# whaiproject/BetaZero

Hardware: AMD Instinct MI355X
Metric: selfplay_games_per_s (higher is better)
Workload: dtype bf16

## Files before the change

betazero_amd/_lib.py:

```python
import ctypes as C
import os

HERE = os.path.dirname(os.path.abspath(__file__))
SO = os.environ.get("BZ_HIP_SO") or os.path.join(HERE, "libbz_hip.so")
ABI_VERSION = 7

BZ_OK, BZ_EINVAL, BZ_EILLEGAL_MOVE, BZ_EHIP, BZ_ENOMEM, BZ_ENOGPU, BZ_ESTATE = range(7)
GAME_TTT, GAME_REVERSI, GAME_REVERSI6, GAME_REVERSI4 = 0, 1, 2, 3
EVAL_UNIFORM, EVAL_HASH, EVAL_NET_F32, EVAL_NET_BF16, EVAL_EXTERNAL, EVAL_NET_FP8, EVAL_MLP_F32, EVAL_MLP_BF16 = range(8)
ST_RUNNING, ST_TERMINAL, ST_ILLEGAL, ST_MUST_PASS = range(4)
PASS_ACTION = 64
ENGINE_REUSE_SUBTREE = 1
ENGINE_EVAL_CACHE = 2
ENGINE_EVAL_CACHE_CARRY = 4
ENGINE_LEAVES_SHIFT = 8
ENGINE_LEAVES_MASK = 31 << ENGINE_LEAVES_SHIFT
PROBE_OPS = ("expf_spec", "logf_spec", "tanhf_spec", "fsqrt", "fdiv", "u01_spec", "hash_logit", "hash_value", "gamma_spec")
PROBE_HOST, PROBE_DEVICE = 0, 1
PROBE_MAP, PROBE_SWEEP = 0, 1
PROF_SLOTS = ("tower", "stem", "heads", "select", "expand_backup", "search_fused", "play", "env_step")
COUNTER_NAMES = ("n_sims", "n_path_nodes", "n_child_scored", "n_edges_backed", "n_expanded",
                 "n_child_written", "n_env_steps", "n_net_leaves", "n_cache_hits", "n_cache_hits_prev", "n_collisions")

u64, u32, i32, i64, vp = C.c_uint64, C.c_uint32, C.c_int32, C.c_int64, C.c_void_p
# ... 87 lines not shown
    "bz_reversi_legal_batch": (i32, [vp, vp, i64, vp, vp]),
    "bz_reversi_score_batch": (i32, [vp, vp, i64, vp, vp, vp]),
    "bz_ttt_step_batch": (i32, [vp, vp, vp, vp, i64, vp, vp, vp, vp, vp, vp]),
    "bz_reversi_minimax": (i32, [u64, u64, i32, i32, C.POINTER(i32), C.POINTER(i32)]),
    "bz_ttt_minimax": (i32, [u32, u32, i32, C.POINTER(i32), C.POINTER(i32)]),
    "bz_reversi_minimax_batch": (i32, [vp, vp, vp, i64, i32, i32, vp, vp, vp]),
    "bz_ttt_minimax_batch": (i32, [vp, vp, vp, vp, i64, vp, vp, vp]),
    "bz_augment_d4_batch": (i32, [vp, vp, vp, i64, i32, i32, vp, vp, vp, vp, vp]),
    "bz_net_update": (i32, [vp, vp, vp]),
    "bz_net_param_count": (i64, [i32, i32, i32]),
    "bz_net_workspace_bytes": (i64, [i32, i32, i32, i32]),
    "bz_net_create": (i32, [i32, i32, i32, i32, vp, vp, i64, vp, C.POINTER(vp)]),
    "bz_net_destroy": (i32, [vp]),
    "bz_net_forward_f32": (i32, [vp, vp, vp, i32, vp, vp, vp]),
    "bz_net_forward_bf16": (i32, [vp, vp, vp, i32, vp, vp, vp]),
    "bz_net_forward_fp8": (i32, [vp, vp, vp, i32, vp, vp, vp]),
    "bz_sym_index": (u32, [u64, u64, u64]),
    "bz_sym_board": (i32, [u64, i32, i32, C.POINTER(u64)]),
    "bz_sym_action_map": (i32, [i32, i32, vp]),
    "bz_net_sym_scratch_bytes": (i64, [i64]),
    "bz_net_forward_sym": (i32, [vp, i32, vp, vp, i32, i32, i32, u64, vp, i64, vp, vp, vp]),
    "bz_net_forward_sym_counted": (i32, [vp, i32, vp, vp, i32, vp, i32, i32, u64, vp, vp, vp]),
    "bz_net_forward_counted": (i32, [vp, i32, vp, vp, i32, vp, vp, vp, vp]),
    "bz_net_set_adaptive_shape": (i32, [vp, i32]),
    "bz_net_shape_tally": (i32, [vp, vp, vp]),
    "bz_net_set_tile_map": (i32, [vp, i32]),
    "bz_mlp_param_count": (i64, [i32]),
    "bz_mlp_workspace_bytes": (i64, [i32, i32]),
    "bz_mlp_create": (i32, [i32, i32, vp, vp, i64, vp, C.POINTER(vp)]),
    "bz_mlp_destroy": (i32, [vp]),
    "bz_mlp_update": (i32, [vp, vp, vp]),
    "bz_mlp_forward_f32": (i32, [vp, vp, vp, i32, vp, vp]),
    "bz_mlp_forward_bf16": (i32, [vp, vp, vp, i32, vp, vp]),
    "bz_mlp_forward_states_f32": (i32, [vp, vp, i32, vp, vp]),
    "bz_mlp_forward_states_bf16": (i32, [vp, vp, i32, vp, vp]),
    "bz_mlp_train_workspace_bytes": (i64, [i32, i32]),
    "bz_mlp_train_step": (i32, [vp, vp, vp, vp, vp, vp, vp, vp, i32, C.POINTER(MlpAdam), vp, i64, vp, vp, vp, vp]),
    "bz_engine_workspace_bytes": (i64, [C.POINTER(EngineCfg)]),
    "bz_engine_create": (i32, [C.POINTER(EngineCfg), vp, i64, C.POINTER(vp)]),
    "bz_engine_destroy": (i32, [vp]),
    "bz_engine_get_layout": (i32, [vp, C.POINTER(EngineLayout)]),
    "bz_engine_set_net": (i32, [vp, vp]),
    "bz_engine_set_mlp": (i32, [vp, vp]),
    "bz_engine_debug_set_search_seq": (i32, [vp, C.c_uint32]),
    "bz_engine_set_eval_symmetry": (i32, [vp, i32, u64]),
    "bz_engine_reset_games": (i32, [vp, vp]),
    "bz_engine_set_roots": (i32, [vp, vp, vp, vp, vp]),
    "bz_engine_search": (i32, [vp, vp]),
    "bz_engine_root_begin": (i32, [vp, vp]),
    "bz_engine_select": (i32, [vp, u32, vp]),
    "bz_engine_evaluate": (i32, [vp, vp]),
    "bz_engine_expand_backup": (i32, [vp, vp]),
    "bz_engine_root_noise": (i32, [vp, vp]),
    "bz_engine_root_stats": (i32, [vp, vp]),
    "bz_engine_play": (i32, [vp, i32, vp]),
    "bz_engine_gumbel_bytes": (i64, [C.POINTER(EngineCfg), i32]),
    "bz_engine_set_gumbel": (i32, [vp, i32, C.c_float, C.c_float, C.c_float, vp, i64, vp]),
    "bz_gumbel_considered_visits": (i32, [i32, i32, vp]),
    "bz_engine_playout_cap_bytes": (i64, [C.POINTER(EngineCfg)]),
    "bz_engine_set_playout_cap": (i32, [vp, i32, u32, vp, i64, vp]),
    "bz_playout_cap_budget": (i32, [u64, u64, u32, i32, i32, u32]),
    "bz_engine_set_forced_playouts": (i32, [vp, C.c_float, i32, vp]),
    "bz_engine_forced_playouts_check": (i32, [C.POINTER(EngineCfg), C.c_float]),
    "bz_forced_prune": (i32, [vp, vp, vp, i32, C.c_float, C.c_float, vp]),
    "bz_engine_gumbel_interior_bytes": (i64, [C.POINTER(EngineCfg)]),
    "bz_engine_set_gumbel_interior": (i32, [vp, i32, vp, i64, vp]),
    "bz_gumbel_interior_pick": (i32, [vp, vp, vp, i32, C.c_float, C.c_float, C.c_float, vp, vp]),
    "bz_engine_fpu_bytes": (i64, [C.POINTER(EngineCfg)]),
    "bz_engine_fpu_check": (i32, [C.POINTER(EngineCfg), C.c_float, C.c_float]),
    "bz_engine_set_fpu": (i32, [vp, i32, C.c_float, C.c_float, vp, i64, vp]),
    "bz_fpu_mass": (u32, [vp, vp, i32]),
    "bz_fpu_value": (C.c_float, [vp, vp, i32, C.c_float, C.c_float]),
    "bz_engine_solver_bytes": (i64, [C.POINTER(EngineCfg)]),
    "bz_engine_solver_check": (i32, [C.POINTER(EngineCfg)]),
    "bz_engine_set_solver": (i32, [vp, i32, vp, i64, vp]),
    "bz_engine_root_proven": (i32, [vp, vp, vp, vp, vp]),
    "bz_solver_node": (i32, [vp, i32]),
    "bz_solver_pick": (i32, [vp, vp, i32, i32, C.c_uint64]),
    "bz_engine_early_stop_bytes": (i64, [C.POINTER(EngineCfg)]),
    "bz_engine_early_stop_check": (i32, [C.POINTER(EngineCfg)]),
    "bz_engine_set_early_stop": (i32, [vp, i32, i32, vp, i64, vp]),
    "bz_engine_stopped": (i32, [vp, vp, vp]),
    "bz_early_stop_decided": (i32, [vp, i32, u32]),
    "bz_engine_surprise_bytes": (i64, [C.POINTER(EngineCfg)]),
    "bz_engine_set_surprise": (i32, [vp, vp, i64, vp]),
    "bz_engine_pack_surprise": (i32, [vp, vp, i64, i32, vp]),
    "bz_surprise_kl": (i32, [vp, vp, i32, vp]),
    "bz_surprise_resample_workspace_bytes": (i64, [i64]),
    "bz_surprise_resample": (i32, [vp, vp, vp, vp, vp, i64, C.c_float, u64, vp, i64, vp, vp, i64, vp, vp]),
    "bz_surprise_count": (i32, [C.c_float, C.c_float, C.c_float, u64, i64, i32, u64, u64, C.POINTER(i32)]),
    "bz_engine_search_value_bytes": (i64, [C.POINTER(EngineCfg)]),
    "bz_engine_set_search_value": (i32, [vp, vp, i64, vp]),
    "bz_engine_pack_search_value": (i32, [vp, vp, i64, i32, vp]),
    "bz_root_value": (i32, [vp, vp, i32, vp]),
    "bz_value_targets": (i32, [vp, vp, vp, vp, vp, i64, C.c_float, C.c_float, vp, vp, vp]),
    "bz_value_targets_segment": (i32, [vp, vp, vp, i32, C.c_float, C.c_float, vp]),
    "bz_merge_group": (i32, [vp, vp, vp, vp, vp, i32, i32, vp, vp, vp, vp, vp, vp]),
    "bz_merge_workspace_bytes": (i64, [i64, i32]),
    "bz_merge_positions": (i32, [C.POINTER(MergeRows), i64, i32, vp, vp, vp, vp, vp, vp, vp, i64, C.POINTER(MergeRows), vp, vp]),
    "bz_engine_ownership_bytes": (i64, [C.POINTER(EngineCfg)]),
    "bz_engine_set_ownership": (i32, [vp, vp, i64, vp]),
    "bz_engine_pack_ownership": (i32, [vp, vp, vp, i64, i32, vp]),
    "bz_ownership_row": (i32, [u64, u64, i32, vp, vp]),
    "bz_engine_resign_bytes": (i64, [C.POINTER(EngineCfg)]),
    "bz_engine_set_resign": (i32, [vp, C.c_float, i32, u32, vp, i64, vp]),
    "bz_engine_resign_rows": (i32, [vp, vp, vp, vp, vp, vp]),
    "bz_resign_step": (i32, [C.c_float, C.c_float, i32, i32, vp]),
    "bz_resign_playout": (i32, [u64, u64, u32]),
    "bz_engine_root_store_bytes": (i64, [C.POINTER(EngineCfg), i32, i32]),
    "bz_engine_set_root_store": (i32, [vp, vp, i64, i32, i32, vp]),
    "bz_engine_root_policy": (i32, [vp, vp, vp, vp]),
    "bz_engine_status": (i32, [vp, vp, C.POINTER(i32), C.POINTER(i64), C.POINTER(i32)]),
    "bz_mcts_select": (i32, [vp, u32, vp]),
    "bz_mcts_expand_backup": (i32, [vp, vp]),
    "bz_selfplay_run": (i32, [vp, i32, vp]),
    "bz_engines_step": (i32, [C.POINTER(vp), C.POINTER(vp), i32, i32, i32]),
    "bz_engines_search": (i32, [C.POINTER(vp), C.POINTER(vp), i32, i32]),
    "bz_match_workspace_bytes": (i64, [i32, i32, i32]),
    "bz_match_create": (i32, [i32, i32, i32, vp, i64, C.POINTER(vp)]),
    "bz_match_destroy": (i32, [vp]),
    "bz_match_get_layout": (i32, [vp, C.POINTER(MatchLayout)]),
    "bz_match_begin": (i32, [vp, u64, i32, vp]),
    "bz_match_ply": (i32, [vp, vp, vp, vp, vp, vp]),
    "bz_match_header": (i32, [vp, vp, C.POINTER(MatchHdr)]),
    "bz_match_opening_index": (i32, [u64, u64, i32, i32, C.POINTER(i32)]),
    "bz_engine_reset_counters": (i32, [vp, vp]),
    "bz_engine_sum_counters": (i32, [vp, vp]),
    "bz_examples_packed_bytes": (i64, [i32, i64]),
    "bz_engine_pack_examples": (i32, [vp, vp, i64, i64, i32, vp]),
    "bz_stream_overlap_probe": (i32, [vp, vp, i32, i32, C.POINTER(C.c_float)]),
    "bz_spec_probe": (i32, [i32, i32, i32, vp, vp, i64, u64, u64, vp, vp]),
    "bz_train_wf_bytes": (i64, [i32, i32]),
    "bz_train_positions_per_workgroup": (i32, [i32]),
    "bz_train_mask_bytes": (i64, [i32, i32, i32]),
    "bz_train_pack_weights": (i32, [vp, i32, i32, vp, vp, vp]),
    "bz_train_tower_fwd": (i32, [vp, vp, vp, i32, i32, i32, vp, vp, vp]),
    "bz_train_tower_bwd": (i32, [vp, vp, vp, vp, i32, i32, i32, vp, vp]),
    "bz_train_wgrad_splits": (i32, [i32, i32, i32]),
    "bz_train_wgrad_bias_rows": (i32, [i32, i32]),
    "bz_train_wgrad": (i32, [vp, vp, i32, i32, i32, i32, vp, vp, vp]),
    "bz_train_ends_sizes": (i32, [i32, i32, C.POINTER(i32)]),
    "bz_train_stem_fwd": (i32, [vp, i32, vp, vp, i32, vp, vp]),
    "bz_train_stem_wgrad": (i32, [vp, vp, vp, i32, i32, vp, vp]),
    "bz_train_heads": (i32, [vp, vp, i32, i32, i32, C.POINTER(TrainHeadParams), vp, vp, vp, vp, vp, vp]),
    "bz_train_heads_vt": (i32, [vp, vp, vp, i32, i32, i32, C.POINTER(TrainHeadParams), vp, vp, vp, vp, vp, vp]),
    "bz_train_heads_own": (i32, [vp, vp, C.POINTER(TrainOwn), i32, i32, i32, C.POINTER(TrainHeadParams), vp, vp, vp, vp, vp, vp]),
    "bz_train_heads_own_vt": (i32, [vp, vp, vp, C.POINTER(TrainOwn), i32, i32, i32, C.POINTER(TrainHeadParams), vp, vp, vp, vp, vp, vp]),
    "bz_train_own_finish": (i32, [C.POINTER(TrainOwn), i32, i32, vp, vp, vp, vp, C.POINTER(TrainOwnAdam), vp]),
    "bz_train_heads_wgrad": (i32, [vp, vp, vp, i32, i32, vp, vp]),
    "bz_train_finish": (i32, [C.POINTER(TrainPartials), C.POINTER(TrainTensors), i32, i32, i32, i32, vp, C.POINTER(TrainAdam), vp]),
    "bz_train_optim_partials": (i32, []),
    "bz_train_optim_hyper": (i32, [C.c_float, C.c_float, C.c_float, C.c_float, C.c_float, C.c_float, C.POINTER(C.c_float)]),
    "bz_train_optim_step": (i32, [C.POINTER(TrainTensors), C.POINTER(TrainOptim), i32, i32, i32, vp]),
    "bz_profile_enable": (i32, [i32]),
    "bz_profile_reserve": (i32, [i32, i64]),
    "bz_profile_read": (i32, [i32, C.POINTER(i64), C.POINTER(i64), C.POINTER(C.c_double)]),
    "bz_profile_reset": (i32, []),
    "bz_profile_intervals": (i32, [i32, vp, vp, i64, C.POINTER(i64)]),
}
ABI_SYMBOLS = tuple(_SIGS)

_lib = None


def lib():
    global _lib
# ... 72 lines not shown
```

betazero_amd/csrc/bz_mcts.hip:

```cpp
#include <new>

#include <time.h>

#include "bz_common.h"
#include "bz_math.h"
#include "bz_rules.h"
#include "bz_fpu.h"
#include "bz_solver.h"
#include "bz_early_stop.h"
#include "bz_gumbel_interior.h"
#include "bz_surprise.h"
#include "bz_value.h"
#include "bz_ownership.h"
#include "bz_resign.h"

using namespace bz;

namespace {

struct __attribute__((aligned(16))) Node { u64 own, opp, legal; u32 edge0, info; };
struct __attribute__((aligned(16))) Edge { u32 w0; float W; float P; u32 w3; };
static_assert(sizeof(Node) == 32 && sizeof(Edge) == 16, "layout");
constexpr int kNBits = 14, kActShift = 14, kNchShift = 21, kTermShift = 27, kValShift = 28, kChildBits = 13;
constexpr u32 kNMask = (1u << kNBits) - 1u, kChildMask = (1u << kChildBits) - 1u;
constexpr int kMaxNodes = (1 << kChildBits) - 1;
__host__ __device__ __forceinline__ u32 e_N(u32 w0) { return w0 & kNMask; }
__host__ __device__ __forceinline__ int e_action(u32 w0) { return (int)((w0 >> kActShift) & 0x7Fu); }
__host__ __device__ __forceinline__ int e_nch(u32 w0) { return (int)((w0 >> kNchShift) & 0x3Fu); }
__host__ __device__ __forceinline__ bool e_term(u32 w0) { return ((w0 >> kTermShift) & 1u) != 0; }
__host__ __device__ __forceinline__ int e_val(u32 w0) { return (int)((w0 >> kValShift) & 3u) - 1; }
constexpr int kProvenShift = 30;
constexpr u32 kProven = 1u << kProvenShift, kDecidedMask = kProven | (1u << kTermShift);
__host__ __device__ __forceinline__ bool e_decided(u32 w0) { return (w0 & kDecidedMask) != 0; }
__host__ __device__ __forceinline__ int e_cval(u32 w0) { return e_decided(w0) ? e_val(w0) : kSolverUndecided; }
__host__ __device__ __forceinline__ u32 e_child(u32 w3) { return w3 & kChildMask; }
__host__ __device__ __forceinline__ u32 e_edge0(u32 w3) { return w3 >> kChildBits; }

constexpr u32 kTerm = 1u << 8;
enum { LEAF_NONE = 0, LEAF_EVAL = 1, LEAF_TERMINAL = 2, LEAF_READY = 3, LEAF_COPY = 4, LEAF_COLLIDE = 5 };
enum { CNT_SIMS, CNT_PATH_NODES, CNT_CHILD_SCORED, CNT_EDGES_BACKED, CNT_EXPANDED, CNT_CHILD_WRITTEN,
       CNT_ENV_STEPS, CNT_NET_LEAVES, CNT_CACHE_HITS, CNT_CACHE_HITS_PREV, CNT_N };
constexpr int kCntCollisions = 10;
constexpr int kCntWords = 24;
enum { FLAG_ERR = 0, FLAG_FINISHED = 1, FLAG_ACTIVE = 2, FLAG_NEVAL = 4, FLAG_N = 8 };
enum { ERR_EDGE_OVERFLOW = 1, ERR_TERMINAL_ROOT = 2, ERR_EXAMPLE_OVERFLOW = 4, ERR_DEPTH = 8, ERR_EVAL_NONFINITE = 16 };

struct __attribute__((aligned(16))) PathEnt { u32 eidx; u32 w0; float W; u32 pad; };

struct __attribute__((aligned(64))) GameHot {
    u64 leaf_legal; u32 leaf_node, leaf_info;
    u32 depth, n_nodes, n_edges, leaf_slot;
    u32 root_n, root_base;
    u32 tt_gen, copy_src, copy_e0, last_gen, prev_nodes, pad[1];
};
constexpr u32 kSrcPrev = 1u << 31;
static_assert(sizeof(GameHot) == 64, "layout");

struct __attribute__((aligned(16))) LeafRec { u64 legal; u32 node, info, slot, depth, kind; float v; };
static_assert(sizeof(LeafRec) == 32, "layout");

struct EngineDev {
    int B, ncap, ecap, sims, na, t_max, rounds, temp_moves, openings, maxd, stagger;
    int compact;
    int reuse;
    Node* nodes_alt; Edge* edges_alt; u32* g_reuse;
    float c_puct, dir_alpha, dir_eps;
    u64 seed, id_base, id_stride;
    Node* nodes; Edge* edges;
    u64 *g_own, *g_opp; int8_t* g_to_move; uint8_t* g_state; int32_t *g_moves, *g_nex, *g_round, *g_passes;
    struct GameHot* hot;
    PathEnt* path;
    int K;
    LeafRec* lrec;
    uint8_t* leaf_kind; u64 *leaf_own, *leaf_opp, *c_own, *c_opp;
    float *logits, *value;
    u64 *ex_own, *ex_opp; float* ex_pi; int8_t *ex_z, *ex_mover; uint8_t* ex_act; int32_t* ex_len; int8_t* ex_winner;
    u32* root_N; float *root_W, *root_P;
    u64* counters; u64* cnt_slots; int n_cnt_slots; u32* flags;
    int32_t* pack_off;
    int ecache, tt_buckets; u64* tt; float *node_v, *node_v_alt;
};

struct GumbelDev {
    int m; float scale, mvi, vs;
    const uint16_t* T; float *base, *vroot;
};

struct CapDev {
    int fast; u32 full_q;
    u32* budget;
};
constexpr u64 kCapKey = 0x706C61796F757443ULL;
__host__ __device__ __forceinline__ u32 cap_budget(u64 seed, u64 gid, u64 made, int sims, int fast, u32 full_q) {
    return (u32)(rng_draw(seed ^ kCapKey, gid, made) & 0xFFFFULL) < full_q ? (u32)sims : (u32)fast;
}

struct ForcedDev { float k; int prune; };
__host__ __device__ __forceinline__ float forced_nf(float k, float P, u32 sumN) {
    float t = k * P;
    t = t * (float)sumN;
    return fsqrt(t);
}
__host__ __device__ __forceinline__ float puct_score(float q, float c_puct, float P, float sq, float Nf) {
    float u = c_puct * P;
    u = u * sq;
    u = fdiv(u, 1.0f + Nf);
    return q + u;
}
template <class Sink>
__host__ __device__ __forceinline__ u32 forced_prune(const Edge* ed, int n, float c_puct, float k, Sink&& sink) {
    u32 sumN = 0, bn = 0;
    int cs = 0;
    for (int i = 0; i < n; ++i) {
        const u32 N = e_N(ed[i].w0);
        sumN += N;
        if (N > bn) { bn = N; cs = i; }
    }
    const float sq = fsqrt((float)(sumN > 1u ? sumN : 1u));
    float ss = 0.0f;
    if (n > 0) {
        const Edge b = ed[cs];
        ss = puct_score(bn > 0 ? fdiv(b.W, (float)bn) : 0.0f, c_puct, b.P, sq, (float)bn);
    }
    u32 sum2 = 0;
    for (int i = 0; i < n; ++i) {
        const Edge e = ed[i];
        const u32 N = e_N(e.w0);
        u32 Np = N;
        if (i != cs && N > 0) {
            const float nf = forced_nf(k, e.P, sumN);
            const u32 lim = !(nf < (float)N) ? N : (u32)__builtin_ceilf(nf);
            const float q = fdiv(e.W, (float)N);
            for (u32 t = 1; t <= lim; ++t) {
                if (!(puct_score(q, c_puct, e.P, sq, (float)(N - t)) < ss)) break;
                Np = N - t;
            }
            if (Np < N && Np <= 1u) Np = 0;
        }
        sink(i, e, Np);
        sum2 += Np;
    }
    return sum2;
}

struct SurpDev { float* prior; u64* pend; float* ex_kl; };
struct ValueDev { float* ex_q; };
struct FpuDev { float reduction, root_reduction; float* root_w; };
struct GumbelInDev { float* node_v; };
struct OwnDev { u64 *fin_x, *fin_o; float* pi; int32_t* act; };

struct SolveDev { int32_t* root; u32* counts; };

struct ResignDev { float threshold; int consecutive; u32 playout_q; uint8_t* streak; int8_t* side; int32_t* move; float* q; uint8_t* played_out; };
constexpr uint8_t kStateResigned = 2;
struct StopDev { u32* stop_at; u32* walked; };

enum : unsigned {
    kModeLeaf = 1u << 0,
    kModeGumbel = 1u << 1,
    kModeCap = 1u << 2,
    kModeForced = 1u << 3,
    kModeFpu = 1u << 4,
    kModeGfull = 1u << 5,
    kModeSolve = 1u << 6,
    kModeStop = 1u << 7,
};
template <unsigned M>
struct Mode {
    static constexpr bool leaf = (M & kModeLeaf) != 0, gumbel = (M & kModeGumbel) != 0, cap = (M & kModeCap) != 0,
                          forced = (M & kModeForced) != 0, fpu = (M & kModeFpu) != 0, gfull = (M & kModeGfull) != 0,
                          solve = (M & kModeSolve) != 0, stop = (M & kModeStop) != 0;
    static_assert(!gfull || gumbel, "search mode: the Gumbel interior rule needs Gumbel root search");
    static_assert(!gumbel || !(cap || forced || fpu || solve),
                  "search mode: Gumbel root search combines with none of playout cap, forced playouts, FPU reduction and the solver");
    static_assert(!solve || !(forced || fpu), "search mode: the solver combines with neither forced playouts nor FPU reduction");
    static_assert(!leaf || M == kModeLeaf, "search mode: leaf-parallel search combines with nothing");
    static_assert(!stop || !(leaf || gumbel || cap || forced || gfull || solve),
                  "search mode: early stop combines with FPU reduction and with nothing else");
};
struct ModeArgs {
    const GumbelDev* gm = nullptr;
    const u32* budget = nullptr;
    const ForcedDev* fo = nullptr;
    const FpuDev* fp = nullptr;
    const GumbelInDev* gi = nullptr;
    const SolveDev* sv = nullptr;
    const StopDev* sp = nullptr;
};

struct Cnt { u32 v[CNT_N]; };

#ifdef BZ_EXP_TREE_STAMPS
struct Stamps {
    u64 last; u32 acc[8];
    __device__ __forceinline__ void start() { for (int k = 0; k < 8; ++k) acc[k] = 0; last = __builtin_readcyclecounter(); }
    __device__ __forceinline__ void mark(int k) { const u64 now = __builtin_readcyclecounter(); acc[k] += (u32)(now - last); last = now; }
    __device__ __forceinline__ void flush(u64* counters) {
        if ((threadIdx.x & 63) == 0) {
            for (int k = 0; k < 7; ++k) atomicAdd(reinterpret_cast<unsigned long long*>(counters) + 16 + k, (unsigned long long)acc[k]);
            atomicAdd(reinterpret_cast<unsigned long long*>(counters) + 23, 1ULL);
        }
    }
};
#else
struct Stamps {
    __device__ __forceinline__ void start() {}
    __device__ __forceinline__ void mark(int) {}
    __device__ __forceinline__ void flush(u64*) {}
};
#endif

template <int O>
__device__ __forceinline__ int xchg_i(int x) {
    static_assert(O == 1 || O == 2 || O == 4 || O == 8, "butterfly step");
    constexpr int ctrl = O == 1 ? 0xB1 : (O == 2 ? 0x4E : (O == 4 ? 0x141 : 0x140));
    return __builtin_amdgcn_update_dpp(0, x, ctrl, 0xF, 0xF, true);
}
template <int O> __device__ __forceinline__ u32 xchg(u32 x) { return (u32)xchg_i<O>((int)x); }
template <int O> __device__ __forceinline__ int xchg(int x) { return xchg_i<O>(x); }
template <int O> __device__ __forceinline__ float xchg(float x) { return __int_as_float(xchg_i<O>(__float_as_int(x))); }
__device__ __forceinline__ float row_shr1(float x) {
    return __int_as_float(__builtin_amdgcn_update_dpp(0, __float_as_int(x), 0x111, 0xF, 0xF, true));
}

struct Cand { float sc; int i; u32 w0, w3; float W; };
template <int O>
__device__ __forceinline__ void cand_step(Cand& c) {
    const float s2 = xchg<O>(c.sc), W2 = xchg<O>(c.W); const int i2 = xchg<O>(c.i);
    const u32 a2 = xchg<O>(c.w0), b2 = xchg<O>(c.w3);
    const bool take = (s2 > c.sc) || (s2 == c.sc && i2 < c.i);
    if (take) { c.sc = s2; c.i = i2; c.w0 = a2; c.w3 = b2; c.W = W2; }
}
template <int kGW>
__device__ __forceinline__ void group_argmax(Cand& c) {
    if (kGW > 1) cand_step<1>(c);
    if (kGW > 2) cand_step<2>(c);
    if (kGW > 4) cand_step<4>(c);
    if (kGW > 8) cand_step<8>(c);
}
template <int kGW>
__device__ __forceinline__ float group_max(float m) {
    if (kGW > 1) { float m2 = xchg<1>(m); m = m2 > m ? m2 : m; }
    if (kGW > 2) { float m2 = xchg<2>(m); m = m2 > m ? m2 : m; }
    if (kGW > 4) { float m2 = xchg<4>(m); m = m2 > m ? m2 : m; }
    if (kGW > 8) { float m2 = xchg<8>(m); m = m2 > m ? m2 : m; }
    return m;
}
template <int kGW>
__device__ __forceinline__ float group_min(float m) {
    if (kGW > 1) { float m2 = xchg<1>(m); m = m2 < m ? m2 : m; }
    if (kGW > 2) { float m2 = xchg<2>(m); m = m2 < m ? m2 : m; }
    if (kGW > 4) { float m2 = xchg<4>(m); m = m2 < m ? m2 : m; }
    if (kGW > 8) { float m2 = xchg<8>(m); m = m2 < m ? m2 : m; }
    return m;
}
template <int kGW>
__device__ __forceinline__ u32 group_max_u32(u32 m) {
    if (kGW > 1) { u32 m2 = xchg<1>(m); m = m2 > m ? m2 : m; }
    if (kGW > 2) { u32 m2 = xchg<2>(m); m = m2 > m ? m2 : m; }
    if (kGW > 4) { u32 m2 = xchg<4>(m); m = m2 > m ? m2 : m; }
    if (kGW > 8) { u32 m2 = xchg<8>(m); m = m2 > m ? m2 : m; }
// ... 756 lines not shown
        const bool carry = E.ecache == 2 && carry_ok && E.hot[g].last_gen == gen_prev;
        E.hot[g].prev_nodes = carry ? E.hot[g].n_nodes : 0u;
        E.hot[g].tt_gen = tt_gen;
        if (E.g_state[g] == 0) E.hot[g].last_gen = tt_gen;
    }
    const u32 keep = (E.reuse && E.g_state[g] == 0) ? E.g_reuse[g] : 0u;
    if (keep) {
        dev_reroot<G>(E, g, keep);
        kind = LEAF_READY;
        E.hot[g].leaf_node = 0; E.hot[g].depth = 0;
    } else if (E.g_state[g] == 0 && dev_root_init<G>(E, g)) {
        kind = LEAF_EVAL;
        E.hot[g].n_nodes = 1; E.hot[g].n_edges = 0; E.hot[g].leaf_node = 0; E.hot[g].depth = 0;
        E.hot[g].root_base = 0;
    }
    const size_t r0 = (size_t)g * E.K;
    E.leaf_own[r0] = E.g_own[g]; E.leaf_opp[r0] = E.g_opp[g];
    E.leaf_kind[r0] = kind;
    u32 slot = 0;
    if (E.compact && kind == LEAF_EVAL) {
        slot = atomicAdd(&E.flags[FLAG_NEVAL + 1], 1u);
        E.hot[g].leaf_slot = slot; E.c_own[slot] = E.g_own[g]; E.c_opp[slot] = E.g_opp[g];
    }
    if (E.K > 1) {
        LeafRec r; r.legal = E.hot[g].leaf_legal; r.node = 0; r.info = E.hot[g].leaf_info; r.slot = slot; r.depth = 0;
        r.kind = kind; r.v = 0.0f;
        E.lrec[r0] = r;
        for (int j = 1; j < E.K; ++j) { E.lrec[r0 + j].kind = LEAF_NONE; E.leaf_kind[r0 + j] = LEAF_NONE; }
    }
    if (g == 0) E.flags[FLAG_NEVAL] = 0;
}

template <bool kCap>
__device__ __forceinline__ void root_noise_body(const EngineDev& E, const u32* budget) {
    const int g = blockIdx.x * blockDim.x + threadIdx.x;
    if (g >= E.B || E.g_state[g] != 0) return;
    if (kCap && budget[g] < (u32)E.sims) return;
    const Node r = E.nodes[(size_t)g * E.ncap];
    const int n = (int)(r.info & 0xFFu);
    if (n == 0 || r.legal == 0) return;
    Edge* ed = E.edges + (size_t)g * E.ecap + r.edge0;
    const u64 gid = E.id_base + (u64)E.g_round[g] * E.id_stride + (u64)g, ply = (u64)E.g_moves[g];
    float gs = 0.0f;
    for (int i = 0; i < n; ++i) gs = gs + gamma_spec(E.dir_alpha, E.seed, gid, ply, i);
    if (!(gs > 0.0f)) return;
    const float keep = 1.0f - E.dir_eps;
    for (int i = 0; i < n; ++i) {
        float t1 = keep * ed[i].P;
        float t2 = E.dir_eps * fdiv(gamma_spec(E.dir_alpha, E.seed, gid, ply, i), gs);
        ed[i].P = t1 + t2;
    }
}
__global__ void __launch_bounds__(64) k_root_noise(EngineDev E) { root_noise_body<false>(E, nullptr); }
__global__ void __launch_bounds__(64) k_cap_noise(EngineDev E, CapDev Cp) { root_noise_body<true>(E, Cp.budget); }

__global__ void __launch_bounds__(256) k_cap_budget(EngineDev E, CapDev Cp) {
    const int g = blockIdx.x * blockDim.x + threadIdx.x;
    if (g >= E.B) return;
    u32 b = 0;
    if (E.g_state[g] == 0) {
        const u64 gid = E.id_base + (u64)E.g_round[g] * E.id_stride + (u64)g;
        b = cap_budget(E.seed, gid, (u64)E.g_moves[g], E.sims, Cp.fast, Cp.full_q);
    }
    Cp.budget[g] = b;
}

template <class G>
__global__ void __launch_bounds__(256) k_eval_synth(EngineDev E, int eval_kind) {
    const int rows = E.B * E.K;
    for (int g = blockIdx.x * blockDim.x + threadIdx.x; g < rows; g += gridDim.x * blockDim.x) {
        if (E.leaf_kind[g] != LEAF_EVAL) continue;
        u64 h = hash_pos(E.leaf_own[g], E.leaf_opp[g]);
        float* row = E.logits + (size_t)g * G::NA;
        for (int a = 0; a < G::NA; ++a) row[a] = eval_kind == BZ_EVAL_HASH ? hash_logit(h, a) : 0.0f;
        E.value[g] = eval_kind == BZ_EVAL_HASH ? hash_value(h) : 0.0f;
    }
}

template <class T> __device__ __forceinline__ void pin(T& x) { asm volatile("" : "+v"(x)); }

template <class G, unsigned M>
__device__ __forceinline__ void tree_step_body(const EngineDev& E, const ModeArgs& A, int do_expand, int do_select, u32 sim_idx) {
    constexpr bool kGumbel = Mode<M>::gumbel, kCap = Mode<M>::cap, kForced = Mode<M>::forced, kFpu = Mode<M>::fpu, kGfull = Mode<M>::gfull,
                   kSolve = Mode<M>::solve, kStop = Mode<M>::stop;
    static_assert(!Mode<M>::leaf, "search mode: the leaf-parallel step is k_leaf_step's own body");
    constexpr int kGW = G::GW;
    const int t = blockIdx.x * blockDim.x + threadIdx.x;
    const int g = t / kGW, sub = t % kGW;
    Cnt c = {};
    Stamps st; st.start();
    __shared__ u32 s_need, s_base;
    if (threadIdx.x == 0) s_need = 0;
    __syncthreads();
    bool want_slot = false; u32 my_rank = 0; u64 slot_own = 0, slot_opp = 0;
    if (g < E.B) {
        PathEnt* path = E.path + (size_t)g * E.maxd;
        int kind = E.leaf_kind[g], state = E.g_state[g];
        const GameHot hot = E.hot[g];
        u32 leaf = hot.leaf_node, ninfo = hot.leaf_info, ne = hot.n_edges, nn = hot.n_nodes, row = E.compact ? hot.leaf_slot : (u32)g;
        int depth0 = (int)hot.depth, root_n = (int)hot.root_n, rtm = E.g_to_move[g];
        u64 nlegal = hot.leaf_legal, rown = E.g_own[g], ropp = E.g_opp[g];
        u32 root_base = E.reuse ? hot.root_base : 0u;
        PathEnt pe0 = path[sub];
        u32 bud = 0;
        if (kCap) { bud = A.budget[g]; pin(bud); }
        [[maybe_unused]] float rw;
        if constexpr (kFpu) { rw = A.fp->root_w[g]; pin(rw); }
        [[maybe_unused]] int made = 0;
        if constexpr (kStop) { made = E.g_moves[g]; pin(made); }
        Edge* const edges_g = E.edges + (size_t)g * E.ecap;
        Edge re0 = edges_g[sub];
        pin(re0.w0); pin(re0.W); pin(re0.P); pin(re0.w3);
        bool pre_ok = true;
        pin(kind); pin(state); pin(leaf); pin(ninfo); pin(ne); pin(nn); pin(row); pin(depth0); pin(root_n); pin(rtm);
        pin(nlegal); pin(rown); pin(ropp); pin(root_base); pin(pe0.eidx); pin(pe0.w0); pin(pe0.W);
        const bool active = state == 0 && kind != LEAF_NONE;
        bool walk = kCap ? (active && sim_idx < bud) : active;
        st.mark(0);
        if (do_expand && (kind == LEAF_EVAL || kind == LEAF_TERMINAL || kind == LEAF_COPY)) {
            float v;
            u32 e0 = ne; int n = 0;
            if (kind == LEAF_EVAL) {
                LogitSrc ls; ls.kind = BZ_EVAL_EXTERNAL; ls.h = 0; ls.row = E.logits + (size_t)row * G::NA;
                v = E.value[row];
                if (sub == 0 && !(v >= -3.0e38f && v <= 3.0e38f)) atomicOr(&E.flags[FLAG_ERR], ERR_EVAL_NONFINITE);
                n = dev_expand<G>(E, g, sub, leaf, nlegal, ninfo, ls, ne, c, st);
                if (sub == 0) {
                    E.hot[g].n_edges = ne; c.v[CNT_NET_LEAVES]++; if (leaf == 0) E.hot[g].root_n = (u32)n;
                    if (E.ecache) E.node_v[(size_t)g * E.ncap + leaf] = v;
                    if (kGumbel && leaf == 0) A.gm->vroot[g] = v;
                    if constexpr (kGfull) A.gi->node_v[(size_t)g * E.ncap + leaf] = v;
                }
                if (leaf == 0) { root_n = n; pre_ok = false; }
            } else if (kind == LEAF_COPY) {
                const bool from_prev = (hot.copy_src & kSrcPrev) != 0u;
                v = (from_prev ? E.node_v_alt : E.node_v)[(size_t)g * E.ncap + (hot.copy_src & ~kSrcPrev)];
                n = dev_expand_copy<G>(E, g, sub, leaf, nlegal, ninfo, hot.copy_e0, from_prev, ne, c);
                if (sub == 0) {
                    E.hot[g].n_edges = ne; E.node_v[(size_t)g * E.ncap + leaf] = v;
                    if (kGumbel && leaf == 0) A.gm->vroot[g] = v;
                    if constexpr (kGfull) A.gi->node_v[(size_t)g * E.ncap + leaf] = v;
                }
            } else {
                v = (float)((int)((ninfo >> 9) & 3u) - 1);
            }
            Edge* edges = edges_g;
            const int dmax = depth0 < E.maxd ? depth0 : E.maxd;
            uint2 wr = make_uint2(0u, 0u);
            if (sub < dmax) wr = backup_edge(edges, pe0, ((dmax - 1 - sub) & 1) ? v : -v, sub == depth0 - 1, leaf, e0, n);
            for (int d = sub + kGW; d < dmax; d += kGW)
                backup_edge(edges, path[d], ((dmax - 1 - d) & 1) ? v : -v, d == depth0 - 1, leaf, e0, n);
            if (sub == 0) c.v[CNT_EDGES_BACKED] += (u32)dmax;
            if constexpr (kFpu) if (dmax >= 1) {
                rw = (sim_idx == 1u ? 0.0f : rw) + (((dmax - 1) & 1) ? v : -v);
                if (sub == 0) A.fp->root_w[g] = rw;
            }
            if (dmax >= 1) {
                const u32 pe_e = (u32)__shfl((int)pe0.eidx, 0, kGW), w0n = (u32)__shfl((int)wr.x, 0, kGW), Wn = (u32)__shfl((int)wr.y, 0, kGW);
                if ((u32)sub == pe_e) {
                    re0.w0 = w0n; re0.W = __uint_as_float(Wn);
                    if (depth0 == 1 && n > 0) re0.w3 = leaf | (e0 << kChildBits);
                }
            }
            if constexpr (kSolve) if (kind == LEAF_TERMINAL) dev_prove<G>(E, *A.sv, g, sub, path, depth0, root_n, re0);
        }
        if constexpr (kStop) {
            const u32 left = (u32)E.sims - sim_idx;
            if (do_select && walk && pre_ok && made >= E.temp_moves && early_stop_possible(root_n, sim_idx, left)) {
                constexpr int kCH = (G::MAXCH + kGW - 1) / kGW;
                group_fence();
                u32 Nk[kCH], key = 0;
#pragma unroll
                for (int k = 0; k < kCH; ++k) {
                    const int i = k * kGW + sub;
                    Nk[k] = 0;
                    if (i < root_n) {
                        Nk[k] = e_N(k == 0 ? re0.w0 : edges_g[i].w0);
                        const u32 ky = early_stop_key(Nk[k], i);
                        key = ky > key ? ky : key;
                    }
                }
                key = group_max_u32<kGW>(key);
                const u32 NL = early_stop_leader_N(key);
                const int L = early_stop_leader(key);
                u32 open = 0;
#pragma unroll
                for (int k = 0; k < kCH; ++k) {
                    const int i = k * kGW + sub;
                    if (i < root_n && early_stop_catches(Nk[k], i, NL, L, left)) open = 1u;
                }
                open = group_or_u32<kGW>(open);
                if (!open) {
                    walk = false;
                    if (sub == 0) A.sp->stop_at[g] = sim_idx;
                }
            }
            if (do_select && walk && sub == 0) A.sp->walked[0] = sim_idx + 1u;
        }
        st.mark(2);
        if (do_select) {
            uint8_t kind8 = LEAF_NONE;
            if (walk) {
                group_fence();
                u32 leaf2; int k2, depth; float tv;
                LeafPos lpos; lpos.own = 0; lpos.opp = 0; lpos.legal = 0; lpos.info = 0; lpos.src = 0; lpos.src_e0 = 0;
                RootRef root; root.own = rown; root.opp = ropp; root.tm = rtm; root.n = root_n;
                root.sumN = sim_idx + root_base; root.has_pre = pre_ok; root.pre = re0; root.tt_gen = hot.tt_gen; root.prev_nodes = hot.prev_nodes;
                PathHbm<kGW> sink; sink.p = path; sink.mine.eidx = 0; sink.mine.w0 = 0; sink.mine.W = 0.0f; sink.mine.pad = 0;
                const float fslot = (kForced && (!kCap || bud >= (u32)E.sims)) ? A.fo->k : 0.0f;
                dev_select<G, M>(E, g, sub, root, nn, leaf2, k2, depth, tv, c, sink, lpos, st, A, fslot, kFpu ? rw : 0.0f);
                sink.flush(sub, depth);
                if (sub == 0) {
                    E.hot[g].n_nodes = nn; E.hot[g].leaf_node = leaf2; E.hot[g].depth = (u32)depth;
                    if (k2 == LEAF_EVAL) {
                        E.leaf_own[g] = lpos.own; E.leaf_opp[g] = lpos.opp; E.hot[g].leaf_legal = lpos.legal; E.hot[g].leaf_info = lpos.info;
                        if (E.compact) { want_slot = true; my_rank = atomicAdd(&s_need, 1u); slot_own = lpos.own; slot_opp = lpos.opp; }
                    } else if (k2 == LEAF_COPY) {
                        E.hot[g].leaf_legal = lpos.legal; E.hot[g].leaf_info = lpos.info;
                        E.hot[g].copy_src = lpos.src; E.hot[g].copy_e0 = lpos.src_e0;
                    } else {
                        E.hot[g].leaf_info = (u32)((int)tv + 1) << 9;
                    }
                }
                kind8 = (uint8_t)k2;
            }
            if (sub == 0) E.leaf_kind[g] = kind8;
            if (t == 0) E.flags[FLAG_NEVAL + ((sim_idx + 1u) & 1u)] = 0;
        } else if (t == 0) {
            E.flags[FLAG_NEVAL] = 0; E.flags[FLAG_NEVAL + 1] = 0;
        }
    }
    if (do_select && E.compact) {
        __syncthreads();
        if (threadIdx.x == 0) s_base = s_need ? atomicAdd(&E.flags[FLAG_NEVAL + (sim_idx & 1u)], s_need) : 0u;
        __syncthreads();
        if (want_slot) {
            const u32 slot = s_base + my_rank;
            E.hot[g].leaf_slot = slot; E.c_own[slot] = slot_own; E.c_opp[slot] = slot_opp;
        }
    }
    st.mark(5);
    cnt_flush<G::GW>(E, c);
    st.mark(6);
    st.flush(E.counters);
}

template <class G>
__global__ void __launch_bounds__(256) k_tree_step(EngineDev E, int do_expand, int do_select, u32 sim_idx) {
    tree_step_body<G, 0u>(E, ModeArgs{}, do_expand, do_select, sim_idx);
}

template <class G>
__global__ void __launch_bounds__(256) k_gumbel_step(EngineDev E, GumbelDev Gm, int do_expand, int do_select, u32 sim_idx) {
    ModeArgs A; A.gm = &Gm;
    tree_step_body<G, kModeGumbel>(E, A, do_expand, do_select, sim_idx);
}

template <class G>
__global__ void __launch_bounds__(256) k_gfull_step(EngineDev E, GumbelDev Gm, GumbelInDev Gi, int do_expand, int do_select, u32 sim_idx) {
    ModeArgs A; A.gm = &Gm; A.gi = &Gi;
    tree_step_body<G, kModeGumbel | kModeGfull>(E, A, do_expand, do_select, sim_idx);
}

template <class G>
__global__ void __launch_bounds__(256) k_cap_step(EngineDev E, CapDev Cp, int do_expand, int do_select, u32 sim_idx) {
    ModeArgs A; A.budget = Cp.budget;
    tree_step_body<G, kModeCap>(E, A, do_expand, do_select, sim_idx);
}

template <class G>
__global__ void __launch_bounds__(256) k_forced_step(EngineDev E, ForcedDev F, int do_expand, int do_select, u32 sim_idx) {
    ModeArgs A; A.fo = &F;
    tree_step_body<G, kModeForced>(E, A, do_expand, do_select, sim_idx);
}
template <class G>
__global__ void __launch_bounds__(256) k_forced_cap_step(EngineDev E, CapDev Cp, ForcedDev F, int do_expand, int do_select, u32 sim_idx) {
    ModeArgs A; A.budget = Cp.budget; A.fo = &F;
    tree_step_body<G, kModeForced | kModeCap>(E, A, do_expand, do_select, sim_idx);
}

template <class G>
__global__ void __launch_bounds__(256) k_fpu_step(EngineDev E, FpuDev Fp, int do_expand, int do_select, u32 sim_idx) {
    ModeArgs A; A.fp = &Fp;
    tree_step_body<G, kModeFpu>(E, A, do_expand, do_select, sim_idx);
}
template <class G>
__global__ void __launch_bounds__(256) k_fpu_cap_step(EngineDev E, CapDev Cp, FpuDev Fp, int do_expand, int do_select, u32 sim_idx) {
    ModeArgs A; A.budget = Cp.budget; A.fp = &Fp;
    tree_step_body<G, kModeFpu | kModeCap>(E, A, do_expand, do_select, sim_idx);
}
template <class G>
__global__ void __launch_bounds__(256) k_fpu_forced_step(EngineDev E, ForcedDev F, FpuDev Fp, int do_expand, int do_select, u32 sim_idx) {
    ModeArgs A; A.fo = &F; A.fp = &Fp;
    tree_step_body<G, kModeFpu | kModeForced>(E, A, do_expand, do_select, sim_idx);
}
template <class G>
__global__ void __launch_bounds__(256) k_fpu_forced_cap_step(EngineDev E, CapDev Cp, ForcedDev F, FpuDev Fp, int do_expand, int do_select,
                                                             u32 sim_idx) {
    ModeArgs A; A.budget = Cp.budget; A.fo = &F; A.fp = &Fp;
    tree_step_body<G, kModeFpu | kModeForced | kModeCap>(E, A, do_expand, do_select, sim_idx);
}

template <class G>
__global__ void __launch_bounds__(256) k_solve_step(EngineDev E, SolveDev Sv, int do_expand, int do_select, u32 sim_idx) {
    ModeArgs A; A.sv = &Sv;
    tree_step_body<G, kModeSolve>(E, A, do_expand, do_select, sim_idx);
}
template <class G>
__global__ void __launch_bounds__(256) k_solve_cap_step(EngineDev E, CapDev Cp, SolveDev Sv, int do_expand, int do_select, u32 sim_idx) {
    ModeArgs A; A.budget = Cp.budget; A.sv = &Sv;
    tree_step_body<G, kModeSolve | kModeCap>(E, A, do_expand, do_select, sim_idx);
}

template <class G>
__global__ void __launch_bounds__(256) k_stop_step(EngineDev E, StopDev Sp, int do_expand, int do_select, u32 sim_idx) {
    ModeArgs A; A.sp = &Sp;
    tree_step_body<G, kModeStop>(E, A, do_expand, do_select, sim_idx);
}
template <class G>
__global__ void __launch_bounds__(256) k_fpu_stop_step(EngineDev E, FpuDev Fp, StopDev Sp, int do_expand, int do_select, u32 sim_idx) {
    ModeArgs A; A.fp = &Fp; A.sp = &Sp;
    tree_step_body<G, kModeFpu | kModeStop>(E, A, do_expand, do_select, sim_idx);
}
__global__ void __launch_bounds__(256) k_stop_begin(EngineDev E, StopDev Sp) {
    const int g = blockIdx.x * blockDim.x + threadIdx.x;
    if (g == 0) Sp.walked[0] = 0u;
    if (g < E.B) Sp.stop_at[g] = E.leaf_kind[(size_t)g * E.K] != LEAF_NONE ? (u32)E.sims : 0u;
}

template <class G>
__global__ void __launch_bounds__(256) k_leaf_step(EngineDev E, int do_expand, int do_select, u32 sim_idx) {
    constexpr int kGW = G::GW;
// ... 796 lines not shown
    const int a = O.act[g];
    if (a < 0 || a >= G::NA) return;
    const bool record = !(budget && budget[g] < (u32)E.sims);
    if (record && E.g_nex[g] >= E.t_max) return;
    const int round = E.g_round[g];
    if (round < 0 || round >= E.rounds) return;
    const Node root = E.nodes[(size_t)g * E.ncap];
    u64 own, opp;
    G::apply(root.own, root.opp, a, &own, &opp);
    const int tm = -(int)E.g_to_move[g];
    const u64 lg = G::legal(own, opp);
    int tv;
    if (!G::terminal(own, opp, tm, lg, &tv)) return;
    const size_t i = (size_t)round * E.B + g;
    O.fin_x[i] = tm == 1 ? own : opp;
    O.fin_o[i] = tm == 1 ? opp : own;
}
template <class G>
__global__ void __launch_bounds__(256) k_resign_note(EngineDev E, ResignDev R, const u32* budget) {
    const int g = blockIdx.x * blockDim.x + threadIdx.x;
    if (g >= E.B || E.g_state[g] != 0) return;
    const int round = E.g_round[g];
    if (round < 0 || round >= E.rounds) return;
    const size_t i = (size_t)round * E.B + g;
    const bool out = resign_played_out(E.seed, E.id_base + (u64)round * E.id_stride + (u64)g, R.playout_q);
    R.played_out[i] = out ? 1 : 0;
    if (budget && budget[g] < (u32)E.sims) return;
    const Node r = E.nodes[(size_t)g * E.ncap];
    const int n = (int)(r.info & 0xFFu);
    if (n == 0) return;
    const Edge* ed = E.edges + (size_t)g * E.ecap + r.edge0;
    const float q = root_value(n, [ed](int k) { return e_N(ed[k].w0); }, [ed](int k) { return ed[k].W; });
    const int tm = E.g_to_move[g];
    uint8_t* st = R.streak + i * 2 + (tm == 1 ? 0 : 1);
    int s;
    const bool fire = resign_step(q, R.threshold, R.consecutive, (int)*st, &s);
    *st = (uint8_t)s;
    if (!fire) return;
    if (R.side[i] == 0) { R.side[i] = (int8_t)tm; R.move[i] = E.g_moves[g]; R.q[i] = q; }
    if (out) return;
    const int nex = E.g_nex[g] < E.t_max ? E.g_nex[g] : E.t_max, w = -tm;
    const size_t rowbase = i * E.t_max;
    for (int t = 0; t < nex; ++t) E.ex_z[rowbase + t] = (int8_t)(w * E.ex_mover[rowbase + t]);
    E.ex_len[i] = nex;
    E.ex_winner[i] = (int8_t)w;
    atomicAdd(&E.flags[FLAG_FINISHED], 1u);
    E.g_state[g] = kStateResigned;
}
template <class G>
__global__ void __launch_bounds__(256) k_resign_finish(EngineDev E, int restart) {
    const int g = blockIdx.x * blockDim.x + threadIdx.x;
    if (g >= E.B || E.g_state[g] != kStateResigned) return;
    const int round = E.g_round[g];
    if (restart && round + 1 < E.rounds) { dev_start_game<G>(E, g, round + 1); return; }
    E.g_state[g] = 1;
}

__global__ void __launch_bounds__(256) k_pack_own(EngineDev E, OwnDev O, u64* fown, u64* fopp, int64_t cap) {
    const int i = (int)blockIdx.x * 4 + (int)(threadIdx.x >> 6), lane = threadIdx.x & 63;
    if (i >= E.rounds * E.B) return;
    const int off = E.pack_off[i];
    if (off < 0) return;
    const int len = E.ex_len[i];
    const size_t src = (size_t)i * E.t_max;
    const u64 fx = O.fin_x[i], fo = O.fin_o[i];
    for (int t = lane; t < len && t < E.t_max && (int64_t)off + t < cap; t += 64) {
        u64 a, b;
        ownership_row(fx, fo, (int)E.ex_mover[src + t], &a, &b);
        fown[(size_t)off + t] = a; fopp[(size_t)off + t] = b;
    }
}

struct __attribute__((aligned(64))) StoreHdr { u64 own, opp, epoch; u32 n_nodes, n_edges, ready, pad[7]; };
static_assert(sizeof(StoreHdr) == 64, "layout");
struct StoreDev {
    int S, D, n_idx, base;
    u32* n_used;
    u32* idx;
    StoreHdr* hdr;
    u32* mark;
    Node* nodes; Edge* edges; float* node_v; u64* tt;
};
constexpr int kCntSeededEvals = 11, kCntSeededSearches = 12, kCntStoreSaves = 13;

__device__ __forceinline__ u32 store_home(const StoreDev& St, u64 own, u64 opp) { return (u32)(hash_pos(own, opp) >> 20) & (u32)(St.n_idx - 1); }
__device__ __forceinline__ int store_find(const StoreDev& St, u64 own, u64 opp, u64 epoch, u32* at) {
    u32 p = store_home(St, own, opp);
    for (int k = 0; k < St.n_idx; ++k, p = (p + 1u) & (u32)(St.n_idx - 1)) {
        const u32 w = St.idx[p];
        if (w == 0u || w > (u32)St.S) { *at = p; return -1; }
        const StoreHdr& h = St.hdr[w - 1u];
        if (h.own == own && h.opp == opp && h.epoch == epoch) { *at = p; return (int)(w - 1u); }
    }
    *at = ~0u;
    return -1;
}
__device__ __forceinline__ bool store_depth_ok(const EngineDev& E, const StoreDev& St, int g) {
    const int d = E.g_moves[g] - St.base;
    return E.g_state[g] == 0 && d >= 0 && d < St.D;
}
__device__ __forceinline__ u32 tt_gen_before(u32 gen) { return gen == 1u ? kTtGenMax - 1u : gen - 1u; }

__device__ __forceinline__ bool tt_replay_from_prev(const EngineDev& E, int g, u32 i, u32 gen, u32 prev_nodes) {
    const Node nd = E.nodes[(size_t)g * E.ncap + i];
    if (nd.info & kTerm) return false;
#ifdef BZ_EXP_TT_WEAK_HASH
    const u64 h = hash_pos(nd.own, nd.opp) & 1u;
#else
    const u64 h = hash_pos(nd.own, nd.opp);
#endif
    const u32 tag = (u32)(h >> 32), gen_prev = tt_gen_before(gen);
    const u64* bucket = E.tt + ((size_t)g * (size_t)E.tt_buckets + (size_t)(h & (u64)(E.tt_buckets - 1))) * 16;
    u32 hit = ~0u;
    for (int s = 0; s < 16; ++s) {
        const u64 e = bucket[s];
        const u32 meta = (u32)(e >> 32), egen = meta >> kChildBits;
        const bool cur = egen == gen && (meta & kChildMask) < i, prv = prev_nodes != 0u && egen == gen_prev;
        if ((cur || prv) && (u32)e == tag) {
            const u32 key = ((prv ? 1u : 0u) << 20) | ((u32)s << 16) | (meta & kChildMask);
            hit = key < hit ? key : hit;
        }
    }
    if (hit == ~0u || (hit >> 20) == 0u) return false;
    const u32 x = hit & kChildMask;
    if (x == 0u || x >= prev_nodes) return false;
    const Node xn = E.nodes_alt[(size_t)g * E.ncap + x];
    return xn.own == nd.own && xn.opp == nd.opp && !(xn.info & kTerm) && (xn.info & 0xFFu) != 0u;
}

__global__ void __launch_bounds__(256) k_store_save(EngineDev E, StoreDev St, u32 gen, u64 epoch, const u32* budget) {
    __shared__ int claim[256];
    __shared__ u32 part[256];
    const int t = threadIdx.x;
    if ((int)blockIdx.x < E.B) {
        const int g = blockIdx.x;
        const GameHot& hot = E.hot[g];
        if (E.g_state[g] != 0 || hot.tt_gen != gen || hot.last_gen != gen || hot.prev_nodes == 0u || St.mark[g] != tt_gen_before(gen)) return;
        const u32 n = hot.n_nodes < (u32)E.ncap ? hot.n_nodes : (u32)E.ncap;
        u32 mine = 0;
        for (u32 i = 1u + (u32)t; i < n; i += 256u) mine += tt_replay_from_prev(E, g, i, gen, hot.prev_nodes) ? 1u : 0u;
        part[t] = mine;
        __syncthreads();
        for (int o = 128; o > 0; o >>= 1) { if (t < o) part[t] += part[t + o]; __syncthreads(); }
        if (t == 0 && part[0]) atomicAdd(reinterpret_cast<unsigned long long*>(E.counters) + kCntSeededEvals, (unsigned long long)part[0]);
        return;
    }
    const size_t ttn = (size_t)E.tt_buckets * 16;
    for (int g0 = 0; g0 < E.B; g0 += 256) {
        const int g = g0 + t;
        int c = -1;
        if (g < E.B && store_depth_ok(E, St, g) && E.hot[g].last_gen == gen && E.hot[g].tt_gen == gen && E.hot[g].n_nodes > 1u &&
            E.hot[g].n_nodes <= (u32)E.ncap && E.hot[g].n_edges <= (u32)E.ecap && !(budget && budget[g] < (u32)E.sims)) {
            const Node r = E.nodes[(size_t)g * E.ncap];
            u32 at;
            if (store_find(St, r.own, r.opp, epoch, &at) < 0) c = -2;
        }
        claim[t] = c;
        __syncthreads();
        if (t == 0) {
            for (int j = 0; j < 256; ++j) {
                if (claim[j] != -2) continue;
                claim[j] = -1;
                const u32 used = *St.n_used;
                if (used >= (u32)St.S) continue;
                const int gj = g0 + j;
                const Node r = E.nodes[(size_t)gj * E.ncap];
                u32 at;
                if (store_find(St, r.own, r.opp, epoch, &at) >= 0 || at == ~0u) continue;
                StoreHdr h{};
                h.own = r.own; h.opp = r.opp; h.epoch = epoch; h.n_nodes = E.hot[gj].n_nodes; h.n_edges = E.hot[gj].n_edges; h.ready = 0u;
                St.hdr[used] = h;
                St.idx[at] = used + 1u;
                *St.n_used = used + 1u;
                __threadfence();
                claim[j] = (int)used;
            }
        }
        __syncthreads();
        for (int j = 0; j < 256; ++j) {
            const int en = claim[j];
            if (en < 0) continue;
            const int gj = g0 + j;
            const u32 nn = St.hdr[en].n_nodes, ne = St.hdr[en].n_edges;
            const uint4* sn = reinterpret_cast<const uint4*>(E.nodes + (size_t)gj * E.ncap);
            uint4* dn = reinterpret_cast<uint4*>(St.nodes + (size_t)en * E.ncap);
            for (u32 k = t; k < nn * 2u; k += 256u) dn[k] = sn[k];
            const uint4* se = reinterpret_cast<const uint4*>(E.edges + (size_t)gj * E.ecap);
            uint4* de = reinterpret_cast<uint4*>(St.edges + (size_t)en * E.ecap);
            for (u32 k = t; k < ne; k += 256u) de[k] = se[k];
            const float* sv = E.node_v + (size_t)gj * E.ncap;
            float* dv = St.node_v + (size_t)en * E.ncap;
            for (u32 k = t; k < nn; k += 256u) dv[k] = sv[k];
            const u64* st = E.tt + (size_t)gj * ttn;
            u64* dt = St.tt + (size_t)en * ttn;
            for (size_t k = t; k < ttn; k += 256) {
                const u64 e = st[k];
                dt[k] = ((u32)(e >> 32) >> kChildBits) == gen ? e : 0ULL;
            }
        }
        __syncthreads();
        if (t == 0)
            for (int j = 0; j < 256; ++j)
                if (claim[j] >= 0) {
                    St.hdr[claim[j]].ready = 1u;
                    atomicAdd(reinterpret_cast<unsigned long long*>(E.counters) + kCntStoreSaves, 1ULL);
                }
        __syncthreads();
    }
}

__global__ void __launch_bounds__(256) k_store_seed(EngineDev E, StoreDev St, u32 gen, u64 epoch) {
    __shared__ int found;
    const int g = blockIdx.x, t = threadIdx.x;
    if (t == 0) {
        int en = -1;
        if (store_depth_ok(E, St, g)) {
            u32 at;
            en = store_find(St, E.g_own[g], E.g_opp[g], epoch, &at);
            if (en >= 0 && (St.hdr[en].ready == 0u || St.hdr[en].n_nodes > (u32)E.ncap || St.hdr[en].n_edges > (u32)E.ecap)) en = -1;
        }
        found = en;
    }
    __syncthreads();
    const int en = found;
    if (en < 0) return;
    const u32 nn = St.hdr[en].n_nodes, ne = St.hdr[en].n_edges;
    const uint4* sn = reinterpret_cast<const uint4*>(St.nodes + (size_t)en * E.ncap);
    uint4* dn = reinterpret_cast<uint4*>(E.nodes + (size_t)g * E.ncap);
    for (u32 k = t; k < nn * 2u; k += 256u) dn[k] = sn[k];
    const uint4* se = reinterpret_cast<const uint4*>(St.edges + (size_t)en * E.ecap);
    uint4* de = reinterpret_cast<uint4*>(E.edges + (size_t)g * E.ecap);
    for (u32 k = t; k < ne; k += 256u) de[k] = se[k];
    const float* sv = St.node_v + (size_t)en * E.ncap;
    float* dv = E.node_v + (size_t)g * E.ncap;
    for (u32 k = t; k < nn; k += 256u) dv[k] = sv[k];
    const size_t ttn = (size_t)E.tt_buckets * 16;
    const u64* st = St.tt + (size_t)en * ttn;
    u64* dt = E.tt + (size_t)g * ttn;
    for (size_t k = t; k < ttn; k += 256) {
        const u64 e = st[k];
        dt[k] = e ? ((e & 0xFFFFFFFFULL) | ((u64)((gen << kChildBits) | ((u32)(e >> 32) & kChildMask)) << 32)) : 0ULL;
    }
    if (t == 0) {
        E.hot[g].n_nodes = nn; E.hot[g].last_gen = gen;
        St.mark[g] = gen;
        atomicAdd(reinterpret_cast<unsigned long long*>(E.counters) + kCntSeededSearches, 1ULL);
    }
}

}

struct bz_engine {
    bz_engine_cfg cfg;
    bz_engine_layout lay;
    EngineDev dev;
    bz_net* net;
    bz_mlp* mlp;
    int64_t bytes;
    int pack_parity;
    int ttt_gw;
    uint32_t search_seq;
    uint64_t eval_epoch;
    hipEvent_t ahead[4];
    int n_ahead;
    GumbelDev gumbel;
    GumbelInDev gin;
    CapDev cap;
    ForcedDev forced;
    SurpDev surp;
    FpuDev fpu;
    int fpu_done;
    SolveDev solve;
    int64_t solve_bytes;
    StopDev stop;
    int stop_host_exit;
    uint32_t* stop_ring;
    ValueDev value;
    OwnDev own;
    ResignDev resign;
    int64_t resign_bytes;
    StoreDev store;
    int64_t store_index_bytes;
    int sym_on;
    uint64_t sym_seed;
};

namespace {
struct Carver {
    int64_t off = 0;
    int64_t take(int64_t bytes) { int64_t o = off; off += (bytes + 255) & ~int64_t(255); return o; }
};

struct Offsets {
    int64_t nodes, edges, nodes_alt, edges_alt, g_reuse, g_own, g_opp, g_to_move, g_state, g_moves, g_nex, g_round, g_passes, hot,
        path, lrec, leaf_kind, leaf_own, leaf_opp, c_own, c_opp, logits, value, ex_own, ex_opp, ex_pi, ex_z, ex_mover,
        ex_act, ex_len, ex_winner, ex_meta, root_N, root_W, root_P, counters, cnt_slots, flags, pack_off, tt, node_v, node_v_alt, total;
    int n_cnt_slots;
    int ncap, ecap, na, maxd;
    int ecache, tt_buckets;
};
inline bool net_eval(int ek) { return ek == BZ_EVAL_NET_F32 || ek == BZ_EVAL_NET_BF16 || ek == BZ_EVAL_NET_FP8; }
inline bool mlp_eval(int ek) { return ek == BZ_EVAL_MLP_F32 || ek == BZ_EVAL_MLP_BF16; }

inline int64_t nodes_per_game(const bz_engine_cfg& c) { return ((c.flags & BZ_ENGINE_REUSE_SUBTREE) ? 4 : 1) * ((int64_t)c.sims + 2); }
inline int leaves_per_step(const bz_engine_cfg& c) { return (int)((c.flags & BZ_ENGINE_LEAVES_MASK) >> BZ_ENGINE_LEAVES_SHIFT) + 1; }
constexpr uint32_t kFlagBits = (1u << 13) - 1u;

bool cfg_ok(const bz_engine_cfg* c) {
    if (c && (c->flags & ~kFlagBits)) return false;
    if (!(c && c->game >= BZ_GAME_TTT && c->game <= BZ_GAME_REVERSI4 && c->n_games > 0 && c->sims >= 1 &&
          c->eval_kind >= 0 && c->eval_kind <= BZ_EVAL_MLP_BF16 && (!mlp_eval(c->eval_kind) || c->game == BZ_GAME_TTT) &&
          c->rounds >= 1 &&
          c->t_max >= 1 && c->dirichlet_eps >= 0.0f && c->dirichlet_eps <= 1.0f &&
          (c->dirichlet_eps == 0.0f || (c->dirichlet_alpha > 0.0f && c->dirichlet_alpha <= 1.0f)) &&
          (c->ttt_lanes == -1 || c->ttt_lanes == 0 || c->ttt_lanes == 1 || c->ttt_lanes == 2 || c->ttt_lanes == 4 ||
           c->ttt_lanes == 8)))
        return false;
    return nodes_per_game(*c) <= kMaxNodes;
}

Offsets carve(const bz_engine_cfg& c) {
    Offsets o{};
    bool ttt = c.game == BZ_GAME_TTT;
    o.na = ttt ? TicTacToe::NA : Reversi::NA;
    o.maxd = ttt ? TicTacToe::MAXD : Reversi::MAXD;
    const bool reuse = (c.flags & BZ_ENGINE_REUSE_SUBTREE) != 0;
    o.ncap = (int)nodes_per_game(c);
    o.ecap = o.ncap * (ttt ? TicTacToe::MAXCH : Reversi::MAXCH);
    int64_t B = c.n_games, R = c.rounds, T = c.t_max;
    const int64_t K = leaves_per_step(c);
    Carver k;
    o.nodes = k.take(B * o.ncap * (int64_t)sizeof(Node));
    o.edges = k.take(B * o.ecap * (int64_t)sizeof(Edge));
    o.ecache = ((c.flags & BZ_ENGINE_EVAL_CACHE) && net_eval(c.eval_kind) && !reuse && K == 1) ? ((c.flags & BZ_ENGINE_EVAL_CACHE_CARRY) ? 2 : 1) : 0;
    const bool two = reuse || o.ecache == 2;
    o.nodes_alt = k.take(two ? B * o.ncap * (int64_t)sizeof(Node) : 0);
    o.edges_alt = k.take(two ? B * o.ecap * (int64_t)sizeof(Edge) : 0);
    o.g_reuse = k.take(reuse ? B * 4 : 0);
    o.g_own = k.take(B * 8); o.g_opp = k.take(B * 8); o.g_to_move = k.take(B); o.g_state = k.take(B);
    o.g_moves = k.take(B * 4); o.g_nex = k.take(B * 4); o.g_round = k.take(B * 4); o.g_passes = k.take(B * 4);
    o.hot = k.take(B * (int64_t)sizeof(GameHot));
    o.path = k.take((int64_t)o.maxd * K * B * (int64_t)sizeof(PathEnt));
    o.lrec = k.take(K > 1 ? K * B * (int64_t)sizeof(LeafRec) : 0);
    o.leaf_kind = k.take(K * B); o.leaf_own = k.take(K * B * 8); o.leaf_opp = k.take(K * B * 8);
    o.c_own = k.take(K * B * 8); o.c_opp = k.take(K * B * 8);
    o.logits = k.take(K * B * o.na * 4); o.value = k.take(K * B * 4);
    o.ex_own = k.take(R * B * T * 8); o.ex_opp = k.take(R * B * T * 8); o.ex_pi = k.take(R * B * T * o.na * 4);
    o.ex_z = k.take(R * B * T); o.ex_mover = k.take(R * B * T); o.ex_act = k.take(R * B * T);
    o.ex_len = k.take(R * B * 4); o.ex_winner = k.take(R * B);
    o.ex_meta = k.take(256);
    o.root_N = k.take(B * o.na * 4); o.root_W = k.take(B * o.na * 4); o.root_P = k.take(B * o.na * 4);
    o.counters = k.take(kCntWords * 8);
    o.n_cnt_slots = (int)((B * 16 + 63) / 64) + 4;
    o.cnt_slots = k.take((int64_t)o.n_cnt_slots * CNT_N * 8);
    o.flags = k.take(FLAG_N * 4);
    o.pack_off = k.take(R * B * 4);
    o.tt_buckets = 16;
    while ((int64_t)o.tt_buckets * 16 < (o.ecache == 2 ? 4 : 2) * (int64_t)o.ncap) o.tt_buckets *= 2;
    o.tt = k.take(o.ecache ? B * o.tt_buckets * 16 * 8 : 0);
    o.node_v = k.take(o.ecache ? B * o.ncap * 4 : 0);
    o.node_v_alt = k.take(o.ecache == 2 ? B * o.ncap * 4 : 0);
    o.total = k.off;
    return o;
}

template <class T> T* at(void* base, int64_t off) { return reinterpret_cast<T*>(static_cast<char*>(base) + off); }
inline dim3 grid_of(int B) { return dim3((B + 255) / 256); }
inline dim3 grid_groups(int B, int gw) { return dim3(((size_t)B * gw + 255) / 256); }
}

#define BZ_LAUNCH_ONE(G, KERNEL, grid, stream, ...) \
    hipLaunchKernelGGL(KERNEL<G>, grid, dim3(256), 0, (hipStream_t)(stream), __VA_ARGS__)
#define BZ_DISPATCH_IMPL(e, KERNEL, GRIDFN, stream, ...)                                                        \
    do {                                                                                                        \
        switch ((e)->cfg.game) {                                                                                \
        case BZ_GAME_TTT: BZ_LAUNCH_ONE(TicTacToe, KERNEL, GRIDFN((e)->dev.B, TicTacToe::GW), stream, __VA_ARGS__); break; \
        case BZ_GAME_REVERSI6: BZ_LAUNCH_ONE(Reversi6, KERNEL, GRIDFN((e)->dev.B, Reversi6::GW), stream, __VA_ARGS__); break; \
        case BZ_GAME_REVERSI4: BZ_LAUNCH_ONE(Reversi4, KERNEL, GRIDFN((e)->dev.B, Reversi4::GW), stream, __VA_ARGS__); break; \
        default: BZ_LAUNCH_ONE(Reversi, KERNEL, GRIDFN((e)->dev.B, Reversi::GW), stream, __VA_ARGS__); break;      \
        }                                                                                                       \
        BZ_LAUNCH_CHECK(#KERNEL);                                                                               \
    } while (0)
inline dim3 grid_lane(int B, int) { return grid_of(B); }
#define BZ_DISPATCH(e, KERNEL, stream, ...) BZ_DISPATCH_IMPL(e, KERNEL, grid_lane, stream, __VA_ARGS__)
#define BZ_DISPATCH_G(e, KERNEL, stream, ...) BZ_DISPATCH_IMPL(e, KERNEL, grid_groups, stream, __VA_ARGS__)

const char* kBadCfg = "bad config (note: sims <= 8189, or <= 2045 with BZ_ENGINE_REUSE_SUBTREE -- the packed edge record, bz_abi.h)";
const char* kBadFlags = "bad config: cfg.flags has bits set above bit 12 (the leaves-per-step field BZ_ENGINE_LEAVES_MASK ends there)";

BZ_EXPORT int64_t bz_engine_workspace_bytes(const bz_engine_cfg* cfg) {
    if (cfg && (cfg->flags & ~kFlagBits)) { set_error("bz_engine_workspace_bytes: %s", kBadFlags); return -1; }
    if (!cfg_ok(cfg)) { set_error("bz_engine_workspace_bytes: %s", kBadCfg); return -1; }
    return carve(*cfg).total;
}

BZ_EXPORT int32_t bz_engine_create(const bz_engine_cfg* cfg, void* ws, int64_t bytes, bz_engine** out) {
    BZ_REQUIRE(ws && out, "bz_engine_create: null pointer");
    if (cfg && (cfg->flags & ~kFlagBits)) { set_error("bz_engine_create: %s", kBadFlags); return BZ_EINVAL; }
    if (!cfg_ok(cfg)) { set_error("bz_engine_create: %s", kBadCfg); return BZ_EINVAL; }
    if (bz_device_count() <= 0) { set_error("bz_engine_create: no HIP device (the engine has no CPU path)"); return BZ_ENOGPU; }
    Offsets o = carve(*cfg);
    if (bytes < o.total) { set_error("bz_engine_create: workspace too small (%lld < %lld)", (long long)bytes, (long long)o.total); return BZ_ENOMEM; }
    BZ_REQUIRE((reinterpret_cast<uintptr_t>(ws) & 255) == 0, "bz_engine_create: workspace must be 256-byte aligned");
    bz_engine* e = new (std::nothrow) bz_engine();
    if (!e) { set_error("out of host memory"); return BZ_ENOMEM; }
    e->cfg = *cfg; e->net = nullptr; e->mlp = nullptr; e->bytes = o.total; e->pack_parity = 1; e->n_ahead = 0; e->search_seq = 0; e->eval_epoch = 0;
    e->sym_on = 0; e->sym_seed = 0;
    e->gumbel = GumbelDev{};
    e->gin = GumbelInDev{};
    e->cap = CapDev{};
    e->forced = ForcedDev{};
    e->surp = SurpDev{};
    e->value = ValueDev{};
    e->own = OwnDev{};
    e->resign = ResignDev{}; e->resign_bytes = 0;
    e->store = StoreDev{}; e->store_index_bytes = 0;
    e->fpu = FpuDev{}; e->fpu_done = 0;
    e->solve = SolveDev{}; e->solve_bytes = 0;
    e->stop = StopDev{}; e->stop_host_exit = 0; e->stop_ring = nullptr;
    e->ttt_gw = cfg->ttt_lanes > 0 ? cfg->ttt_lanes : (cfg->ttt_lanes < 0 ? 0 : 4);
    EngineDev& d = e->dev;
    d.B = cfg->n_games; d.ncap = o.ncap; d.ecap = o.ecap; d.sims = cfg->sims; d.na = o.na; d.t_max = cfg->t_max;
    d.rounds = cfg->rounds; d.temp_moves = cfg->temp_moves; d.openings = cfg->openings; d.maxd = o.maxd;
    d.stagger = cfg->stagger;
    d.c_puct = cfg->c_puct; d.dir_alpha = cfg->dirichlet_alpha; d.dir_eps = cfg->dirichlet_eps; d.seed = cfg->seed; d.id_base = cfg->game_id_base; d.id_stride = cfg->game_id_stride;
    d.nodes = at<Node>(ws, o.nodes); d.edges = at<Edge>(ws, o.edges);
    d.reuse = (cfg->flags & BZ_ENGINE_REUSE_SUBTREE) ? 1 : 0;
    d.nodes_alt = at<Node>(ws, o.nodes_alt); d.edges_alt = at<Edge>(ws, o.edges_alt);
    d.g_reuse = at<u32>(ws, o.g_reuse);
    d.g_own = at<u64>(ws, o.g_own); d.g_opp = at<u64>(ws, o.g_opp); d.g_to_move = at<int8_t>(ws, o.g_to_move);
    d.g_state = at<uint8_t>(ws, o.g_state); d.g_moves = at<int32_t>(ws, o.g_moves); d.g_nex = at<int32_t>(ws, o.g_nex);
    d.g_round = at<int32_t>(ws, o.g_round); d.g_passes = at<int32_t>(ws, o.g_passes);
    d.hot = at<GameHot>(ws, o.hot); d.path = at<PathEnt>(ws, o.path);
    d.K = leaves_per_step(*cfg); d.lrec = at<LeafRec>(ws, o.lrec);
    d.leaf_kind = at<uint8_t>(ws, o.leaf_kind);
    d.leaf_own = at<u64>(ws, o.leaf_own); d.leaf_opp = at<u64>(ws, o.leaf_opp);
    d.c_own = at<u64>(ws, o.c_own); d.c_opp = at<u64>(ws, o.c_opp);
    d.compact = (net_eval(cfg->eval_kind) || mlp_eval(cfg->eval_kind)) ? 1 : 0;
    d.ecache = o.ecache; d.tt_buckets = o.tt_buckets; d.tt = at<u64>(ws, o.tt); d.node_v = at<float>(ws, o.node_v); d.node_v_alt = at<float>(ws, o.node_v_alt);
    if (o.ecache) {
        hipError_t ce = hipMemset(d.tt, 0, (size_t)cfg->n_games * o.tt_buckets * 16 * 8);
        if (ce != hipSuccess) { delete e; return hip_fail(ce, "bz_engine_create: evaluation-cache clear"); }
    }
    d.logits = at<float>(ws, o.logits); d.value = at<float>(ws, o.value);
    d.ex_own = at<u64>(ws, o.ex_own); d.ex_opp = at<u64>(ws, o.ex_opp); d.ex_pi = at<float>(ws, o.ex_pi);
    d.ex_z = at<int8_t>(ws, o.ex_z); d.ex_mover = at<int8_t>(ws, o.ex_mover); d.ex_act = at<uint8_t>(ws, o.ex_act);
    d.ex_len = at<int32_t>(ws, o.ex_len); d.ex_winner = at<int8_t>(ws, o.ex_winner);
    d.root_N = at<u32>(ws, o.root_N); d.root_W = at<float>(ws, o.root_W); d.root_P = at<float>(ws, o.root_P);
    d.counters = at<u64>(ws, o.counters); d.flags = at<u32>(ws, o.flags);
    d.cnt_slots = at<u64>(ws, o.cnt_slots); d.n_cnt_slots = o.n_cnt_slots;
    d.pack_off = at<int32_t>(ws, o.pack_off);
    bz_engine_layout& l = e->lay;
    l.ex_own = o.ex_own; l.ex_opp = o.ex_opp; l.ex_pi = o.ex_pi; l.ex_z = o.ex_z; l.ex_mover = o.ex_mover;
    l.ex_act = o.ex_act; l.ex_len = o.ex_len; l.ex_winner = o.ex_winner; l.root_N = o.root_N; l.root_W = o.root_W;
    l.root_P = o.root_P; l.leaf_own = o.leaf_own; l.leaf_opp = o.leaf_opp; l.leaf_kind = o.leaf_kind;
    l.logits = o.logits; l.value = o.value; l.g_own = o.g_own; l.g_opp = o.g_opp; l.g_to_move = o.g_to_move;
    l.g_state = o.g_state; l.counters = o.counters; l.na = o.na; l.t_max = cfg->t_max;
    l.ex_begin = o.ex_own; l.ex_bytes = o.ex_meta + 256 - o.ex_own; l.ex_meta = o.ex_meta;
    {
        uint64_t meta[32] = {0};
        meta[0] = 0x425A455841000002ULL;
        meta[1] = cfg->game_id_base; meta[2] = cfg->game_id_stride; meta[3] = (uint64_t)cfg->n_games;
        meta[4] = (uint64_t)cfg->rounds; meta[5] = (uint64_t)cfg->t_max; meta[6] = (uint64_t)o.na; meta[7] = (uint64_t)cfg->game;
        const int64_t offs[8] = {o.ex_own, o.ex_opp, o.ex_pi, o.ex_z, o.ex_mover, o.ex_act, o.ex_len, o.ex_winner};
        for (int i = 0; i < 8; ++i) meta[8 + i] = (uint64_t)(offs[i] - o.ex_own);
        hipError_t me = hipMemcpy(at<char>(ws, o.ex_meta), meta, sizeof(meta), hipMemcpyHostToDevice);
        if (me != hipSuccess) { delete e; return hip_fail(me, "bz_engine_create: example header upload"); }
    }
    *out = e;
    return BZ_OK;
}

BZ_EXPORT int32_t bz_engine_destroy(bz_engine* e) {
    if (e) for (int i = 0; i < e->n_ahead; ++i) (void)hipEventDestroy(e->ahead[i]);
    if (e && e->stop_ring) (void)hipHostFree(e->stop_ring);
    delete e;
    return BZ_OK;
}

BZ_EXPORT int32_t bz_engine_get_layout(const bz_engine* e, bz_engine_layout* out) {
    BZ_REQUIRE(e && out, "bz_engine_get_layout: null pointer");
    *out = e->lay;
    return BZ_OK;
}

BZ_EXPORT int32_t bz_engine_set_net(bz_engine* e, bz_net* net) {
    BZ_REQUIRE(e, "bz_engine_set_net: null engine");
    BZ_REQUIRE(e->dev.K == 1 || !net || (int64_t)bz_net_max_batch(net) >= (int64_t)e->dev.K * e->dev.B,
               "bz_engine_set_net: the net's max_batch is below leaves_per_step x n_games (the evaluator rows of one step)");
    e->net = net;
    return BZ_OK;
}

BZ_EXPORT int32_t bz_engine_set_mlp(bz_engine* e, bz_mlp* mlp) {
    BZ_REQUIRE(e, "bz_engine_set_mlp: null engine");
    BZ_REQUIRE(e->dev.K == 1 || !mlp || (int64_t)bz_mlp_max_batch(mlp) >= (int64_t)e->dev.K * e->dev.B,
               "bz_engine_set_mlp: the MLP's max_batch is below leaves_per_step x n_games (the evaluator rows of one step)");
    e->mlp = mlp;
    return BZ_OK;
}

BZ_EXPORT int32_t bz_engine_set_eval_symmetry(bz_engine* e, int32_t on, uint64_t seed) {
    BZ_REQUIRE(e, "bz_engine_set_eval_symmetry: null engine");
    on = on != 0;
    if (!on) seed = 0;
    BZ_REQUIRE(!on || (net_eval(e->cfg.eval_kind) && e->cfg.game != BZ_GAME_TTT),
               "bz_engine_set_eval_symmetry: the evaluation symmetry serves the net_f32 / net_bf16 / net_fp8 evaluators on the Reversi boards");
    if (on != e->sym_on || seed != e->sym_seed) e->eval_epoch = 0;
    e->sym_on = on; e->sym_seed = seed;
    return BZ_OK;
}

BZ_EXPORT int32_t bz_engine_debug_set_search_seq(bz_engine* e, uint32_t seq) {
    BZ_REQUIRE(e, "null engine");
    BZ_REQUIRE(seq < kTtGenMax - 1u, "bz_engine_debug_set_search_seq: 0 <= seq <= 2^19 - 3");
    e->search_seq = seq;
    e->eval_epoch = 0;
    return BZ_OK;
}

BZ_EXPORT int32_t bz_engine_reset_counters(bz_engine* e, void* stream) {
    BZ_REQUIRE(e, "null engine");
    BZ_HIP(hipMemsetAsync(e->dev.counters, 0, kCntWords * 8, (hipStream_t)stream));
    BZ_HIP(hipMemsetAsync(e->dev.cnt_slots, 0, (size_t)e->dev.n_cnt_slots * CNT_N * 8, (hipStream_t)stream));
    return BZ_OK;
}

BZ_EXPORT int32_t bz_engine_sum_counters(bz_engine* e, void* stream) {
    BZ_REQUIRE(e, "null engine");
    hipLaunchKernelGGL(k_sum_counters, dim3(1), dim3(256), 0, (hipStream_t)stream, e->dev);
    BZ_LAUNCH_CHECK("k_sum_counters");
    return BZ_OK;
}

BZ_EXPORT int32_t bz_engine_reset_games(bz_engine* e, void* stream) {
    BZ_REQUIRE(e, "null engine");
    BZ_DISPATCH(e, k_reset_games, stream, e->dev);
    if (e->own.fin_x)
        BZ_HIP(hipMemsetAsync(e->own.fin_x, 0, (size_t)(reinterpret_cast<char*>(e->own.pi) - reinterpret_cast<char*>(e->own.fin_x)),
                              (hipStream_t)stream));
    if (e->resign.streak)
        BZ_HIP(hipMemsetAsync(e->resign.streak, 0, (size_t)e->resign_bytes, (hipStream_t)stream));
    return BZ_OK;
}

BZ_EXPORT int32_t bz_engine_set_roots(bz_engine* e, const uint64_t* own, const uint64_t* opp, const int8_t* to_move,
                                      void* stream) {
    BZ_REQUIRE(e && own && opp && to_move, "bz_engine_set_roots: null pointer");
    hipLaunchKernelGGL(k_set_roots, grid_of(e->dev.B), dim3(256), 0, (hipStream_t)stream, e->dev, own, opp, to_move);
    BZ_LAUNCH_CHECK("k_set_roots");
    return BZ_OK;
}

BZ_EXPORT int32_t bz_engine_root_begin(bz_engine* e, void* stream) {
    BZ_REQUIRE(e, "null engine");
    const uint64_t epoch = bz_net_epoch(e->net);
    const int carry_ok = epoch == e->eval_epoch;
    e->eval_epoch = epoch;
    if (e->store.S > 0) {
        if (!carry_ok) BZ_HIP(hipMemsetAsync(e->store.n_used, 0, (size_t)e->store_index_bytes, (hipStream_t)stream));
        else if (e->search_seq != 0u) {
            hipLaunchKernelGGL(k_store_seed, dim3(e->dev.B), dim3(256), 0, (hipStream_t)stream, e->dev, e->store, e->search_seq, epoch);
            BZ_LAUNCH_CHECK("k_store_seed");
        }
    }
    e->search_seq = e->search_seq % (kTtGenMax - 1u) + 1u;
    if (e->dev.ecache == 2) {
        Node* tn = e->dev.nodes; e->dev.nodes = e->dev.nodes_alt; e->dev.nodes_alt = tn;
        Edge* te = e->dev.edges; e->dev.edges = e->dev.edges_alt; e->dev.edges_alt = te;
        float* tv = e->dev.node_v; e->dev.node_v = e->dev.node_v_alt; e->dev.node_v_alt = tv;
    }
    BZ_DISPATCH(e, k_root_begin, stream, e->dev, e->search_seq, carry_ok);
    if (e->cap.fast > 0) {
        hipLaunchKernelGGL(k_cap_budget, grid_of(e->dev.B), dim3(256), 0, (hipStream_t)stream, e->dev, e->cap);
        BZ_LAUNCH_CHECK("k_cap_budget");
    }
    e->pack_parity = 1;
    e->fpu_done = 0;
    if (e->solve.root)
        BZ_HIP(hipMemsetAsync(e->solve.root, 0, (size_t)e->solve_bytes, (hipStream_t)stream));
    if (e->stop.stop_at) {
        hipLaunchKernelGGL(k_stop_begin, grid_of(e->dev.B), dim3(256), 0, (hipStream_t)stream, e->dev, e->stop);
        BZ_LAUNCH_CHECK("k_stop_begin");
    }
    return BZ_OK;
}

static unsigned engine_mode(const bz_engine* e) {
    return (e->dev.K > 1 ? kModeLeaf : 0u) | (e->gumbel.m > 0 ? kModeGumbel : 0u) | (e->cap.fast > 0 ? kModeCap : 0u) |
           (e->forced.k > 0.0f ? kModeForced : 0u) | (e->fpu.root_w ? kModeFpu : 0u) | (e->gin.node_v ? kModeGfull : 0u) |
           (e->solve.root ? kModeSolve : 0u) | (e->stop.stop_at ? kModeStop : 0u);
}
static const u32* cap_budgets(const bz_engine* e) { return e->cap.fast > 0 ? static_cast<const u32*>(e->cap.budget) : nullptr; }

static int32_t tree_step(bz_engine* e, int do_expand, int do_select, uint32_t sim_idx, void* stream) {
    ProfScope ps(do_select ? BZ_PROF_SELECT : BZ_PROF_EXPAND_BACKUP, stream);
    const unsigned m = engine_mode(e);
    if ((m & kModeFpu) && !do_select) sim_idx = (uint32_t)e->fpu_done;
#define BZ_STEP(KERNEL, ...) BZ_DISPATCH_G(e, KERNEL, stream, __VA_ARGS__, do_expand, do_select, sim_idx); break
    switch (m) {
    case 0u: BZ_STEP(k_tree_step, e->dev);
    case kModeLeaf: BZ_STEP(k_leaf_step, e->dev);
    case kModeGumbel: BZ_STEP(k_gumbel_step, e->dev, e->gumbel);
    case kModeGumbel | kModeGfull: BZ_STEP(k_gfull_step, e->dev, e->gumbel, e->gin);
    case kModeCap: BZ_STEP(k_cap_step, e->dev, e->cap);
    case kModeForced: BZ_STEP(k_forced_step, e->dev, e->forced);
    case kModeForced | kModeCap: BZ_STEP(k_forced_cap_step, e->dev, e->cap, e->forced);
    case kModeFpu: BZ_STEP(k_fpu_step, e->dev, e->fpu);
    case kModeFpu | kModeCap: BZ_STEP(k_fpu_cap_step, e->dev, e->cap, e->fpu);
    case kModeFpu | kModeForced: BZ_STEP(k_fpu_forced_step, e->dev, e->forced, e->fpu);
    case kModeFpu | kModeForced | kModeCap: BZ_STEP(k_fpu_forced_cap_step, e->dev, e->cap, e->forced, e->fpu);
    case kModeSolve: BZ_STEP(k_solve_step, e->dev, e->solve);
    case kModeSolve | kModeCap: BZ_STEP(k_solve_cap_step, e->dev, e->cap, e->solve);
    case kModeStop: BZ_STEP(k_stop_step, e->dev, e->stop);
    case kModeFpu | kModeStop: BZ_STEP(k_fpu_stop_step, e->dev, e->fpu, e->stop);
    default: set_error("tree_step: no step kernel serves search mode 0x%x", m); return BZ_EINVAL;
    }
#undef BZ_STEP
    if (do_select) {
        e->pack_parity = (int)(((m & kModeLeaf) ? sim_idx / (uint32_t)e->dev.K : sim_idx) & 1u);
        if (m & kModeFpu) e->fpu_done = (int)sim_idx + 1;
    }
    return BZ_OK;
}

BZ_EXPORT int32_t bz_engine_select(bz_engine* e, uint32_t sim_index, void* stream) {
    BZ_REQUIRE(e, "null engine");
    BZ_REQUIRE(e->dev.K == 1 || (sim_index % (uint32_t)e->dev.K == 0 && sim_index < (uint32_t)e->cfg.sims),
               "bz_engine_select: sim_index must be a multiple of leaves_per_step below sims");
    return tree_step(e, 0, 1, sim_index, stream);
}

BZ_EXPORT int32_t bz_engine_evaluate(bz_engine* e, void* stream) {
    BZ_REQUIRE(e, "null engine");
    int ek = e->cfg.eval_kind;
    if (ek == BZ_EVAL_UNIFORM || ek == BZ_EVAL_HASH) {
        BZ_DISPATCH(e, k_eval_synth, stream, e->dev, ek);
        return BZ_OK;
    }
    if (ek == BZ_EVAL_EXTERNAL) return BZ_OK;
    if (mlp_eval(ek)) {
        BZ_REQUIRE(e->mlp, "bz_engine_evaluate: eval_kind needs an MLP (bz_engine_set_mlp)");
        return bz_mlp_forward_dev(e->mlp, ek == BZ_EVAL_MLP_BF16 ? 1 : 0, e->dev.c_own, e->dev.c_opp, nullptr, e->dev.B * e->dev.K,
                                  e->dev.flags + FLAG_NEVAL + e->pack_parity, e->dev.logits, e->dev.value, stream);
    }
    BZ_REQUIRE(e->net, "bz_engine_evaluate: eval_kind needs a net (bz_engine_set_net)");
    BZ_REQUIRE(e->cfg.game != BZ_GAME_TTT, "bz_engine_evaluate: the conv net serves the Reversi boards, not tic-tac-toe");
    const int kind = ek == BZ_EVAL_NET_BF16 ? 1 : (ek == BZ_EVAL_NET_FP8 ? 2 : 0);
    if (e->sym_on)
        return bz_net_forward_sym_dev(e->net, kind, e->dev.c_own, e->dev.c_opp, e->dev.B * e->dev.K, e->dev.flags + FLAG_NEVAL + e->pack_parity,
                                      e->cfg.game == BZ_GAME_REVERSI6 ? 6 : (e->cfg.game == BZ_GAME_REVERSI4 ? 4 : 8), BZ_SYM_HASHED,
                                      e->sym_seed, nullptr, 0, e->dev.logits, e->dev.value, stream);
    return bz_net_forward_dev(e->net, ek == BZ_EVAL_NET_BF16 ? 1 : (ek == BZ_EVAL_NET_FP8 ? 2 : 0), e->dev.c_own, e->dev.c_opp, e->dev.B * e->dev.K,
                              e->dev.flags + FLAG_NEVAL + e->pack_parity, e->dev.logits, e->dev.value, stream);
}

BZ_EXPORT int32_t bz_engine_expand_backup(bz_engine* e, void* stream) {
    BZ_REQUIRE(e, "null engine");
    return tree_step(e, 1, 0, 0, stream);
}

BZ_EXPORT int32_t bz_engine_root_noise(bz_engine* e, void* stream) {
    BZ_REQUIRE(e, "null engine");
    if (e->surp.prior && e->dev.dir_eps > 0.0f) BZ_DISPATCH(e, k_surp_save, stream, e->dev, e->surp);
    if (e->gumbel.m > 0) BZ_DISPATCH(e, k_gumbel_root, stream, e->dev, e->gumbel);
    if (!(e->dev.dir_eps > 0.0f)) return BZ_OK;
    if (e->cap.fast > 0) {
        hipLaunchKernelGGL(k_cap_noise, dim3((e->dev.B + 63) / 64), dim3(64), 0, (hipStream_t)stream, e->dev, e->cap);
        BZ_LAUNCH_CHECK("k_cap_noise");
        return BZ_OK;
    }
    hipLaunchKernelGGL(k_root_noise, dim3((e->dev.B + 63) / 64), dim3(64), 0, (hipStream_t)stream, e->dev);
    BZ_LAUNCH_CHECK("k_root_noise");
    return BZ_OK;
}

static bool root_prep(const bz_engine* e) { return e->dev.dir_eps > 0.0f || e->gumbel.m > 0; }
static bool search_is_fused(const bz_engine* e) {
    const int ek = e->cfg.eval_kind;
    return (ek == BZ_EVAL_UNIFORM || ek == BZ_EVAL_HASH) && !e->dev.reuse && !root_prep(e) && engine_mode(e) == 0u;
}

static int32_t store_save(bz_engine* e, void* stream) {
    if (e->store.S == 0) return BZ_OK;
    hipLaunchKernelGGL(k_store_save, dim3(e->dev.B + 1), dim3(256), 0, (hipStream_t)stream, e->dev, e->store, e->search_seq, e->eval_epoch,
                       cap_budgets(e));
    BZ_LAUNCH_CHECK("k_store_save");
    return BZ_OK;
}

BZ_EXPORT int32_t bz_engine_search(bz_engine* e, void* stream) {
    BZ_REQUIRE(e, "null engine");
    int ek = e->cfg.eval_kind;
    const bool noise = root_prep(e);
    if (search_is_fused(e)) {
        ProfScope ps(BZ_PROF_SEARCH_FUSED, stream);
        if (e->cfg.game == BZ_GAME_TTT && e->cfg.sims <= kTttFusedMaxSims && e->ttt_gw > 0) {
            const dim3 grid = grid_groups(e->dev.B, e->ttt_gw);
#define BZ_TTT_FUSED(GWN)                                                                                              \
    do {                                                                                                                \
        if (ek == BZ_EVAL_UNIFORM) hipLaunchKernelGGL((k_search_fused_ttt<GWN, true>), grid, dim3(256), 0, (hipStream_t)stream, e->dev); \
        else hipLaunchKernelGGL((k_search_fused_ttt<GWN, false>), grid, dim3(256), 0, (hipStream_t)stream, e->dev);     \
    } while (0)
            switch (e->ttt_gw) {
            case 1: BZ_TTT_FUSED(1); break;
            case 2: BZ_TTT_FUSED(2); break;
            case 8: BZ_TTT_FUSED(8); break;
            default: BZ_TTT_FUSED(4); break;
            }
#undef BZ_TTT_FUSED
            BZ_LAUNCH_CHECK("k_search_fused_ttt");
            return BZ_OK;
        }
        BZ_DISPATCH_G(e, k_search_fused, stream, e->dev, ek);
        return BZ_OK;
    }
    BZ_REQUIRE(ek != BZ_EVAL_EXTERNAL, "bz_engine_search: BZ_EVAL_EXTERNAL callers drive the step API");
    int32_t rc;
    if ((rc = bz_engine_root_begin(e, stream)) != BZ_OK) return rc;
    if ((rc = bz_engine_evaluate(e, stream)) != BZ_OK) return rc;
    if (noise) {
        if ((rc = tree_step(e, 1, 0, 0, stream)) != BZ_OK) return rc;
        if ((rc = bz_engine_root_noise(e, stream)) != BZ_OK) return rc;
    }
    for (int s = 0; s < e->cfg.sims; s += e->dev.K) {
        if ((rc = tree_step(e, (noise && s == 0) ? 0 : 1, 1, (uint32_t)s, stream)) != BZ_OK) return rc;
        if ((rc = bz_engine_evaluate(e, stream)) != BZ_OK) return rc;
    }
    if ((rc = tree_step(e, 1, 0, 0, stream)) != BZ_OK) return rc;
    return store_save(e, stream);
}

BZ_EXPORT int32_t bz_engine_root_stats(bz_engine* e, void* stream) {
    BZ_REQUIRE(e, "null engine");
    BZ_DISPATCH(e, k_root_stats, stream, e->dev);
    return BZ_OK;
}

BZ_EXPORT int32_t bz_gumbel_considered_visits(int32_t n_considered, int32_t sims, uint16_t* out) {
    BZ_REQUIRE(out, "bz_gumbel_considered_visits: null pointer");
    BZ_REQUIRE(n_considered >= 1 && n_considered <= BZ_GUMBEL_MAX_CONSIDERED && sims >= 1 && sims <= BZ_ENGINE_MAX_SIMS,
               "bz_gumbel_considered_visits: n_considered must be in 1..64 and sims in 1..8189");
    if (n_considered <= 1) {
        for (int k = 0; k < sims; ++k) out[k] = (uint16_t)k;
        return BZ_OK;
    }
    int log2max = 0;
    while ((1 << log2max) < n_considered) ++log2max;
    int visits[BZ_GUMBEL_MAX_CONSIDERED] = {0};
    int len = 0, nc = n_considered;
    while (len < sims) {
        const int q = sims / (log2max * nc), extra = q > 1 ? q : 1;
        for (int r = 0; r < extra; ++r) {
            for (int i = 0; i < nc; ++i) {
                if (len < sims) out[len] = (uint16_t)visits[i];
                ++len;
            }
            for (int i = 0; i < nc; ++i) visits[i]++;
        }
        nc = nc / 2 > 2 ? nc / 2 : 2;
    }
    return BZ_OK;
}

namespace {
struct GumbelOffsets { int64_t T, base, vroot, total; };
GumbelOffsets gumbel_carve(const bz_engine_cfg& c, int m) {
    GumbelOffsets o{};
    Carver k;
    const int64_t B = c.n_games, maxch = c.game == BZ_GAME_TTT ? TicTacToe::MAXCH : Reversi::MAXCH;
    o.T = k.take((int64_t)m * c.sims * 2);
    o.base = k.take(B * maxch * 4);
    o.vroot = k.take(B * 4);
    o.total = k.off;
    return o;
}
const char* gumbel_refusal(const bz_engine_cfg& c) {
    if (c.flags & BZ_ENGINE_REUSE_SUBTREE) return "Gumbel root search does not combine with subtree reuse (BZ_ENGINE_REUSE_SUBTREE)";
    if (leaves_per_step(c) > 1) return "Gumbel root search does not combine with leaves_per_step > 1 (BZ_ENGINE_LEAVES_*)";
    if (c.dirichlet_eps > 0.0f) return "Gumbel root search does not combine with Dirichlet noise (dirichlet_eps > 0)";
    return nullptr;
}
}

BZ_EXPORT int64_t bz_engine_gumbel_bytes(const bz_engine_cfg* cfg, int32_t max_considered) {
    if (cfg && (cfg->flags & ~kFlagBits)) { set_error("bz_engine_gumbel_bytes: %s", kBadFlags); return -1; }
    if (!cfg_ok(cfg)) { set_error("bz_engine_gumbel_bytes: %s", kBadCfg); return -1; }
    if (max_considered < 1 || max_considered > BZ_GUMBEL_MAX_CONSIDERED) {
        set_error("bz_engine_gumbel_bytes: max_considered must be in 1..64 (got %d)", (int)max_considered);
        return -1;
    }
    if (const char* why = gumbel_refusal(*cfg)) { set_error("bz_engine_gumbel_bytes: %s", why); return -1; }
    return gumbel_carve(*cfg, max_considered).total;
}

BZ_EXPORT int32_t bz_engine_set_gumbel(bz_engine* e, int32_t max_considered, float gumbel_scale, float maxvisit_init,
                                       float value_scale, void* buf, int64_t buf_bytes, void* stream) {
    BZ_REQUIRE(e, "bz_engine_set_gumbel: null engine");
    if (max_considered == 0) {
        e->gumbel.m = 0;
        e->gin = GumbelInDev{};
        return BZ_OK;
    }
    BZ_REQUIRE(max_considered >= 1 && max_considered <= BZ_GUMBEL_MAX_CONSIDERED, "bz_engine_set_gumbel: max_considered must be in 0..64");
    const bool finite = __builtin_isfinite(gumbel_scale) && __builtin_isfinite(maxvisit_init) && __builtin_isfinite(value_scale);
    BZ_REQUIRE(finite && gumbel_scale >= 0.0f && maxvisit_init >= 0.0f && value_scale >= 0.0f,
               "bz_engine_set_gumbel: gumbel_scale, maxvisit_init and value_scale must be finite and >= 0");
    if (const char* why = gumbel_refusal(e->cfg)) { set_error("bz_engine_set_gumbel: %s", why); return BZ_EINVAL; }
    BZ_REQUIRE(!e->stop.stop_at, "bz_engine_set_gumbel: Gumbel root search does not combine with early stop (bz_engine_set_early_stop)");
    BZ_REQUIRE(e->cap.fast == 0, "bz_engine_set_gumbel: Gumbel root search does not combine with playout cap randomisation (bz_engine_set_playout_cap)");
    BZ_REQUIRE(!(e->forced.k > 0.0f), "bz_engine_set_gumbel: Gumbel root search does not combine with forced playouts (bz_engine_set_forced_playouts)");
    BZ_REQUIRE(!e->fpu.root_w, "bz_engine_set_gumbel: Gumbel root search does not combine with first-play urgency reduction (bz_engine_set_fpu)");
// ... 671 lines not shown
    BZ_HIP(hipMemsetAsync(e->dev.flags + FLAG_ACTIVE, 0, 4, s));
    hipLaunchKernelGGL(k_count_active, grid_of(e->dev.B), dim3(256), 0, s, e->dev);
    BZ_LAUNCH_CHECK("k_count_active");
    u32 h[FLAG_N];
    BZ_HIP(hipMemcpyAsync(h, e->dev.flags, sizeof(h), hipMemcpyDeviceToHost, s));
    BZ_HIP(hipStreamSynchronize(s));
    if (n_active) *n_active = (int32_t)h[FLAG_ACTIVE];
    if (games_finished) *games_finished = (int64_t)h[FLAG_FINISHED];
    if (error_flags) *error_flags = (int32_t)h[FLAG_ERR];
    return BZ_OK;
}



namespace {
PackedLayout packed_layout(int na, int64_t cap) {
    PackedLayout L{};
    Carver k;
    k.take(256);
    const int64_t esz[8] = {8, 8, 4 * (int64_t)na, 8, 1, 1, 1, 1};
    for (int i = 0; i < 8; ++i) L.offs[i] = k.take(cap * esz[i]);
    L.total = k.off;
    return L;
}
}

BZ_EXPORT int64_t bz_examples_packed_bytes(int32_t na, int64_t cap_rows) {
    if (na < 1 || na > 4096 || cap_rows < 1 || cap_rows > (int64_t(1) << 31) - 1) { set_error("bz_examples_packed_bytes: bad arguments"); return -1; }
    return packed_layout(na, cap_rows).total;
}

BZ_EXPORT int32_t bz_engine_pack_examples(bz_engine* e, void* packed, int64_t packed_bytes, int64_t cap_rows, int32_t append,
                                          void* stream) {
    BZ_REQUIRE(e && packed, "bz_engine_pack_examples: null pointer");
    BZ_REQUIRE(cap_rows >= 1 && cap_rows <= (int64_t(1) << 31) - 1, "bz_engine_pack_examples: bad capacity");
    BZ_REQUIRE((reinterpret_cast<uintptr_t>(packed) & 255) == 0, "bz_engine_pack_examples: the block must be 256-byte aligned");
    const PackedLayout L = packed_layout(e->dev.na, cap_rows);
    if (packed_bytes < L.total) { set_error("bz_engine_pack_examples: block too small (%lld < %lld)", (long long)packed_bytes, (long long)L.total); return BZ_ENOMEM; }
    hipLaunchKernelGGL(k_pack_scan, dim3(1), dim3(1024), 0, (hipStream_t)stream, e->dev, static_cast<PackedHdr*>(packed), L,
                       (u64)cap_rows, (int)(append != 0), (int)e->cfg.game);
    BZ_LAUNCH_CHECK("k_pack_scan");
    const int n = e->dev.rounds * e->dev.B;
    hipLaunchKernelGGL(k_pack_rows, dim3((n + 3) / 4), dim3(256), 0, (hipStream_t)stream, e->dev, static_cast<char*>(packed), L);
    BZ_LAUNCH_CHECK("k_pack_rows");
    return BZ_OK;
}

BZ_EXPORT int32_t bz_mcts_select(bz_engine* e, uint32_t sim_index, void* stream) { return bz_engine_select(e, sim_index, stream); }
BZ_EXPORT int32_t bz_mcts_expand_backup(bz_engine* e, void* stream) { return bz_engine_expand_backup(e, stream); }
BZ_EXPORT int32_t bz_selfplay_run(bz_engine* e, int32_t restart, void* stream) {
    int32_t rc = bz_engine_search(e, stream);
    return rc != BZ_OK ? rc : bz_engine_play(e, restart, stream);
}

static int32_t ahead_mark(bz_engine* e, int idx, hipStream_t s) {
    while (e->n_ahead < 4) {
        BZ_HIP(hipEventCreateWithFlags(&e->ahead[e->n_ahead], hipEventBlockingSync | hipEventDisableTiming));
        e->n_ahead++;
    }
    BZ_HIP(hipEventRecord(e->ahead[idx & 3], s));
    if (idx >= 2) {
        const timespec nap = {0, 100 * 1000};
        for (;;) {
            const hipError_t q = hipEventQuery(e->ahead[(idx - 2) & 3]);
            if (q == hipSuccess) break;
            if (q != hipErrorNotReady) return hip_fail(q, "bz_engines_step: hipEventQuery");
            (void)hipGetLastError();
            nanosleep(&nap, nullptr);
        }
    }
    return BZ_OK;
}

static int32_t engines_run(bz_engine* const* engines, void* const* streams, int n, int run_ahead_sims, bool play, int restart) {
    int32_t rc;
    int steps = 0, Kmax = 1;
    for (int i = 0; i < n; ++i) {
        bz_engine* e = engines[i];
        if (!e || search_is_fused(e)) continue;
        const int ns = (e->cfg.sims + e->dev.K - 1) / e->dev.K;
        steps = ns > steps ? ns : steps;
        Kmax = e->dev.K > Kmax ? e->dev.K : Kmax;
        if ((rc = bz_engine_root_begin(e, streams[i])) != BZ_OK) return rc;
        if ((rc = bz_engine_evaluate(e, streams[i])) != BZ_OK) return rc;
        if (root_prep(e)) {
            if ((rc = tree_step(e, 1, 0, 0, streams[i])) != BZ_OK) return rc;
            if ((rc = bz_engine_root_noise(e, streams[i])) != BZ_OK) return rc;
        }
    }
    for (int i = 0; i < n; ++i) {
        bz_engine* e = engines[i];
        if (!e || !search_is_fused(e)) continue;
        if ((rc = bz_engine_search(e, streams[i])) != BZ_OK) return rc;
        if (play && (rc = bz_engine_play(e, restart, streams[i])) != BZ_OK) return rc;
    }
    const int q0 = run_ahead_sims > 0 ? (run_ahead_sims >= 2 ? run_ahead_sims / 2 : 1) : 0;
    const int q = q0 ? (q0 / Kmax > 0 ? q0 / Kmax : 1) : 0;
    bool quit[16] = {};
    for (int step = 0; step < steps; ++step) {
        int live = 0;
        for (int i = 0; i < n; ++i) {
            bz_engine* e = engines[i];
            if (!e || search_is_fused(e) || quit[i]) continue;
            const int s = step * e->dev.K;
            if (s >= e->cfg.sims) continue;
            ++live;
            const bool prep = root_prep(e);
            if ((rc = tree_step(e, (prep && s == 0) ? 0 : 1, 1, (uint32_t)s, streams[i])) != BZ_OK) return rc;
            if ((rc = bz_engine_evaluate(e, streams[i])) != BZ_OK) return rc;
        }
        if (!live) break;
        if (q && (step + 1) % q == 0)
            for (int i = 0; i < n; ++i) {
                bz_engine* e = engines[i];
                if (!e || search_is_fused(e) || quit[i]) continue;
                const int idx = (step + 1) / q - 1;
                const bool watch = !play && e->stop.stop_at && e->stop_host_exit;
                if (watch) {
                    if (!e->stop_ring) BZ_HIP(hipHostMalloc(reinterpret_cast<void**>(&e->stop_ring), 4 * sizeof(uint32_t), hipHostMallocDefault));
                    BZ_HIP(hipMemcpyAsync(e->stop_ring + (idx & 3), e->stop.walked, 4, hipMemcpyDeviceToHost, (hipStream_t)streams[i]));
                }
                if ((rc = ahead_mark(e, idx, (hipStream_t)streams[i])) != BZ_OK) return rc;
                if (watch && idx >= 2 && (int)e->stop_ring[(idx - 2) & 3] <= (idx - 1) * q - 1) quit[i] = true;
            }
    }
    for (int i = 0; i < n; ++i) {
        bz_engine* e = engines[i];
        if (!e || search_is_fused(e)) continue;
        if ((rc = tree_step(e, 1, 0, 0, streams[i])) != BZ_OK) return rc;
        if ((rc = store_save(e, streams[i])) != BZ_OK) return rc;
        if (play && (rc = bz_engine_play(e, restart, streams[i])) != BZ_OK) return rc;
    }
    return BZ_OK;
}

BZ_EXPORT int32_t bz_engines_step(bz_engine* const* engines, void* const* streams, int32_t n, int32_t restart,
                                  int32_t run_ahead_sims) {
    BZ_REQUIRE(engines && streams && n >= 1 && n <= 16 && run_ahead_sims >= 0, "bz_engines_step: bad arguments");
    bool stepwise = true;
    for (int i = 0; i < n; ++i) {
        BZ_REQUIRE(engines[i], "bz_engines_step: null engine");
        BZ_REQUIRE(engines[i]->cfg.sims == engines[0]->cfg.sims, "bz_engines_step: the engines must search the same number of simulations");
        BZ_REQUIRE(engines[i]->dev.K == engines[0]->dev.K, "bz_engines_step: the engines must take the same leaves per step");
        BZ_REQUIRE((engines[i]->gumbel.m > 0) == (engines[0]->gumbel.m > 0),
                   "bz_engines_step: the engines must all search with Gumbel root search or all without");
        BZ_REQUIRE((engines[i]->gin.node_v != nullptr) == (engines[0]->gin.node_v != nullptr),
                   "bz_engines_step: the engines must all search with the Gumbel interior rule or all without");
        BZ_REQUIRE(engines[i]->cfg.eval_kind != BZ_EVAL_EXTERNAL, "bz_engines_step: BZ_EVAL_EXTERNAL callers drive the step API");
        if (search_is_fused(engines[i])) stepwise = false;
    }
    if (!stepwise) {
        int32_t rc;
        for (int i = 0; i < n; ++i)
            if ((rc = bz_selfplay_run(engines[i], restart, streams[i])) != BZ_OK) return rc;
        return BZ_OK;
    }
    return engines_run(engines, streams, n, run_ahead_sims, true, restart);
}

BZ_EXPORT int32_t bz_engines_search(bz_engine* const* engines, void* const* streams, int32_t n, int32_t run_ahead_sims) {
    BZ_REQUIRE(engines && streams && n >= 1 && n <= 16 && run_ahead_sims >= 0, "bz_engines_search: bad arguments");
    for (int i = 0; i < n; ++i)
        BZ_REQUIRE(!engines[i] || engines[i]->cfg.eval_kind != BZ_EVAL_EXTERNAL,
                   "bz_engines_search: BZ_EVAL_EXTERNAL callers drive the step API");
    return engines_run(engines, streams, n, run_ahead_sims, false, 0);
}

const uint32_t* bz_engine_error_word_dev(const bz_engine* e) { return e->dev.flags + FLAG_ERR; }
```

betazero_amd/engine.py:

```python
import ctypes as C
from dataclasses import dataclass

import numpy as np
import torch

from . import _lib
from .symmetry import EvalSymmetry, check_eval_symmetry
from ._lib import (EVAL_EXTERNAL, EVAL_HASH, EVAL_NET_BF16, EVAL_NET_F32, EVAL_NET_FP8, EVAL_UNIFORM, GAME_REVERSI,
                   GAME_REVERSI4, GAME_REVERSI6, GAME_TTT, EngineCfg, EngineLayout)

_GAMES = {"ttt": GAME_TTT, "tic_tac_toe": GAME_TTT, "reversi": GAME_REVERSI, "reversi8": GAME_REVERSI,
          "reversi6": GAME_REVERSI6, "reversi4": GAME_REVERSI4, GAME_TTT: GAME_TTT, GAME_REVERSI: GAME_REVERSI,
          GAME_REVERSI6: GAME_REVERSI6, GAME_REVERSI4: GAME_REVERSI4}
_SIZES = {GAME_TTT: 3, GAME_REVERSI: 8, GAME_REVERSI6: 6, GAME_REVERSI4: 4}
_EVALS = {"uniform": EVAL_UNIFORM, "hash": EVAL_HASH, "net_f32": EVAL_NET_F32, "net_bf16": EVAL_NET_BF16,
          "external": EVAL_EXTERNAL, "net_fp8": EVAL_NET_FP8,
          "mlp_f32": _lib.EVAL_MLP_F32, "mlp_bf16": _lib.EVAL_MLP_BF16}


_EVAL_NAMES = {v: k for k, v in _EVALS.items()}


def _u64(t):
    return t.cpu().numpy().view(np.uint64)
# ... 64 lines not shown
                              z=t(ex.z.astype(np.int8)), mover=t(ex.mover.astype(np.int8)), act=t(ex.act.astype(np.uint8)),
                              game=t(np.asarray(ex.game, np.int64)), ply=t(np.asarray(ex.ply, np.int32)), size=ex.size,
                              kl=None if ex.kl is None else t(np.asarray(ex.kl, np.float32)),
                              q=None if ex.q is None else t(np.asarray(ex.q, np.float32)),
                              vt=None if ex.vt is None else t(np.asarray(ex.vt, np.float32)),
                              fown=None if ex.fown is None else t(np.asarray(ex.fown, np.uint64).view(np.int64)),
                              fopp=None if ex.fopp is None else t(np.asarray(ex.fopp, np.uint64).view(np.int64)))

    def states(self):
        s = self.size
        stride = 3 if s == 3 else 8
        sh = torch.tensor([[stride * r + c for c in range(s)] for r in range(s)], dtype=torch.int64, device=self.own.device)
        a = ((self.own[:, None, None] >> sh) & 1).to(torch.int8)
        b = ((self.opp[:, None, None] >> sh) & 1).to(torch.int8)
        return a - b


_OPTIONAL_FIELDS = (("kl", "policy surprise"), ("q", "search value"), ("vt", "value target"), ("fown", "ownership target"),
                    ("fopp", "ownership target"))


def _all_or_none(parts, field, what):
    have = [getattr(p, field) is not None for p in parts]
    if any(have) and not all(have):
        raise ValueError(f"concatenating examples: every part must carry {field} ({what}), or none")
    return all(have) and len(have) > 0


def concat_device_examples(parts):
    cat = lambda f: torch.cat([getattr(p, f) for p in parts])
    return DeviceExamples(cat("own"), cat("opp"), cat("pi"), cat("z"), cat("mover"), cat("act"), cat("game"), cat("ply"),
                          parts[0].size, *(cat(f) if _all_or_none(parts, f, what) else None for f, what in _OPTIONAL_FIELDS))


MAX_SIMS, MAX_SIMS_REUSE = 8189, 2045


def check_sims(sims, reuse_subtree=False):
    lim = MAX_SIMS_REUSE if reuse_subtree else MAX_SIMS
    if not 1 <= int(sims) <= lim:
        raise ValueError(f"sims must be in 1..{lim}" + (" with subtree reuse" if reuse_subtree else "") +
                         f" (got {sims}): the tree's packed edge record holds at most 8191 nodes per game "
                         "(BZ_ENGINE_MAX_SIMS / BZ_ENGINE_MAX_SIMS_REUSE in include/bz_abi.h)")


MAX_LEAVES_PER_STEP = 32


def check_leaves_per_step(leaves_per_step):
    k = leaves_per_step
    if isinstance(k, bool) or not isinstance(k, (int, np.integer)) or not 1 <= int(k) <= MAX_LEAVES_PER_STEP:
        raise ValueError(f"leaves_per_step must be an int in 1..{MAX_LEAVES_PER_STEP} (got {k!r})")
    return int(k)


EVAL_CACHE_MODES = (True, "carry", "search", False, None)


def check_eval_cache(eval_cache):
    if not any(eval_cache is m or (isinstance(m, str) and isinstance(eval_cache, str) and eval_cache == m)
               for m in EVAL_CACHE_MODES):
        raise ValueError(f"eval_cache must be one of True, 'carry', 'search', False, None (got {eval_cache!r})")
    return eval_cache


ROOT_STORE_DEFAULT = (256, 3)


def check_root_store(root_store, eval_cache=True):
    carry = eval_cache is True or (isinstance(eval_cache, str) and eval_cache == "carry")
    if root_store is None:
        return ROOT_STORE_DEFAULT if carry else None
    if root_store is False:
        return None
    ok = (isinstance(root_store, (tuple, list)) and len(root_store) == 2 and
          all(isinstance(v, (int, np.integer)) and not isinstance(v, (bool, np.bool_)) for v in root_store) and
          1 <= root_store[0] <= 65536 and 1 <= root_store[1] <= 64)
    if not ok:
        raise ValueError(f"root_store must be None, False or (entries in 1..65536, plies in 1..64) (got {root_store!r})")
    return (int(root_store[0]), int(root_store[1])) if carry else None


MAX_CONSIDERED = 64


@dataclass(frozen=True)
class GumbelConfig:
    max_considered: int = 16
    scale: float = 1.0
    maxvisit_init: float = 50.0
    value_scale: float = 0.1
    interior: str = "puct"


GUMBEL_INTERIORS = ("puct", "gumbel")


def check_gumbel(gumbel, reuse_subtree=False, leaves_per_step=1, dirichlet_eps=0.0):
    if gumbel is None or gumbel is False:
        return None
    cfg = GumbelConfig() if gumbel is True else gumbel
    if not isinstance(cfg, GumbelConfig):
        raise ValueError(f"gumbel must be None, False, True or a GumbelConfig (got {gumbel!r})")
    m = cfg.max_considered
    if isinstance(m, bool) or not isinstance(m, (int, np.integer)) or not 1 <= int(m) <= MAX_CONSIDERED:
        raise ValueError(f"gumbel: max_considered must be an int in 1..{MAX_CONSIDERED} (got {m!r})")
    for name in ("scale", "maxvisit_init", "value_scale"):
        x = getattr(cfg, name)
        if isinstance(x, bool) or not isinstance(x, (int, float, np.integer, np.floating)) or not np.isfinite(x) or x < 0:
            raise ValueError(f"gumbel: {name} must be a finite number >= 0 (got {x!r})")
    if not isinstance(cfg.interior, str) or cfg.interior not in GUMBEL_INTERIORS:
        raise ValueError(f"gumbel: interior must be 'puct' or 'gumbel' (got {cfg.interior!r})")
    if reuse_subtree:
        raise ValueError("gumbel: Gumbel root search does not combine with reuse_subtree")
    if leaves_per_step != 1:
        raise ValueError("gumbel: Gumbel root search does not combine with leaves_per_step > 1")
    if dirichlet_eps > 0:
        raise ValueError("gumbel: Gumbel root search does not combine with Dirichlet noise (dirichlet_eps > 0)")
    return GumbelConfig(int(m), float(cfg.scale), float(cfg.maxvisit_init), float(cfg.value_scale), str(cfg.interior))


@dataclass(frozen=True)
class PlayoutCap:
    fast_sims: int
    full_prob: float = 0.25

    @property
    def full_q(self):
        return int(round(float(self.full_prob) * 65536))


def check_playout_cap(playout_cap, sims=None, reuse_subtree=False, leaves_per_step=1, gumbel=None):
    if playout_cap is None or playout_cap is False:
        return None
    cap = playout_cap
    if not isinstance(cap, PlayoutCap):
        raise ValueError(f"playout_cap must be None, False or a PlayoutCap (got {playout_cap!r})")
    n = cap.fast_sims
    if isinstance(n, bool) or not isinstance(n, (int, np.integer)) or n < 1 or (sims is not None and n >= int(sims)):
        raise ValueError(f"playout_cap: fast_sims must be an int in 1..sims - 1 (got {n!r}" +
                         (f", sims = {sims})" if sims is not None else ")"))
    p = cap.full_prob
    if isinstance(p, bool) or not isinstance(p, (int, float, np.integer, np.floating)) or not 0.0 <= p <= 1.0:
        raise ValueError(f"playout_cap: full_prob must be a number in [0, 1] (got {p!r})")
    if reuse_subtree:
        raise ValueError("playout_cap: playout cap randomisation does not combine with reuse_subtree")
    if leaves_per_step != 1:
        raise ValueError("playout_cap: playout cap randomisation does not combine with leaves_per_step > 1")
    if gumbel is not None and gumbel is not False:
        raise ValueError("playout_cap: playout cap randomisation does not combine with Gumbel root search (gumbel)")
    return PlayoutCap(int(n), float(p))


@dataclass(frozen=True)
class Resign:
    threshold: float = -0.9
    consecutive: int = 2
    playout_frac: float = 0.1

    @property
    def playout_q(self):
        return int(round(float(self.playout_frac) * 65536))


def check_resign(resign, ownership=False):
    if resign is None or resign is False:
# ... 85 lines not shown
        out.append(x32)
    if reuse_subtree:
        raise ValueError("fpu: first-play urgency reduction does not combine with reuse_subtree")
    if leaves_per_step != 1:
        raise ValueError("fpu: first-play urgency reduction does not combine with leaves_per_step > 1")
    if gumbel is not None and gumbel is not False:
        raise ValueError("fpu: first-play urgency reduction does not combine with Gumbel root search (gumbel)")
    return Fpu(*out)


def check_solver(solver, reuse_subtree=False, leaves_per_step=1, gumbel=None, forced_playouts=None, fpu=None):
    if solver is None:
        return False
    if not isinstance(solver, (bool, np.bool_)):
        raise ValueError(f"solver must be a bool (got {solver!r})")
    if not solver:
        return False
    if reuse_subtree:
        raise ValueError("solver: proofs do not combine with reuse_subtree")
    if leaves_per_step != 1:
        raise ValueError("solver: proofs do not combine with leaves_per_step > 1 (concurrent walks race on proofs)")
    if gumbel is not None and gumbel is not False:
        raise ValueError("solver: proofs do not combine with Gumbel root search (gumbel)")
    if forced_playouts is not None and forced_playouts is not False:
        raise ValueError("solver: proofs do not combine with forced_playouts (both score +inf)")
    if fpu is not None and fpu is not False:
        raise ValueError("solver: proofs do not combine with first-play urgency reduction (fpu)")
    return True


@dataclass(frozen=True)
class EarlyStop:
    host_exit: bool = True


def check_early_stop(early_stop, reuse_subtree=False, leaves_per_step=1, gumbel=None, playout_cap=None, forced_playouts=None,
                     solver=False, root_store=None, surprise=False, search_value=False, ownership=False, resign=None):
    if early_stop is None or early_stop is False:
        return None
    cfg = EarlyStop() if early_stop is True else early_stop
    if not isinstance(cfg, EarlyStop):
        raise ValueError(f"early_stop must be None, False, True or an EarlyStop (got {early_stop!r})")
    if not isinstance(cfg.host_exit, (bool, np.bool_)):
        raise ValueError(f"early_stop: host_exit must be a bool (got {cfg.host_exit!r})")
    on = lambda x: x is not None and x is not False
    if reuse_subtree:
        raise ValueError("early_stop: early stop does not combine with reuse_subtree")
    if leaves_per_step != 1:
        raise ValueError("early_stop: early stop does not combine with leaves_per_step > 1")
    if on(gumbel):
        raise ValueError("early_stop: early stop does not combine with Gumbel root search (gumbel): sequential halving is its own schedule")
    if on(playout_cap):
        raise ValueError("early_stop: early stop does not combine with playout cap randomisation (playout_cap)")
    if on(forced_playouts):
        raise ValueError("early_stop: early stop does not combine with forced_playouts")
    if on(solver):
        raise ValueError("early_stop: early stop does not combine with the solver (solver)")
    if on(root_store):
        raise ValueError("early_stop: early stop does not combine with the root store (root_store): a shortened tree must not "
                         "seed a later search")
    for name, val in (("surprise", surprise), ("search_value", search_value), ("ownership", ownership), ("resign", resign)):
        if on(val):
            raise ValueError(f"early_stop: early stop does not combine with {name}: its targets come from complete searches")
    return EarlyStop(bool(cfg.host_exit))


def check_search_value(search_value):
    if not isinstance(search_value, (bool, np.bool_)):
        raise ValueError(f"search_value must be a bool (got {search_value!r})")
    return bool(search_value)


def check_ownership(ownership):
    if not isinstance(ownership, (bool, np.bool_)):
        raise ValueError(f"ownership must be a bool (got {ownership!r})")
    return bool(ownership)


class SelfPlayEngine:
    def __init__(self, game, n_games, sims, evaluator="uniform", net=None, c_puct=1.5, temp_moves=0, openings=0,
                 seed=0, rounds=1, game_id_base=0, game_id_stride=None, device="cuda:0", stagger=0,
                 dirichlet_alpha=0.0, dirichlet_eps=0.0, reuse_subtree=False, ttt_lanes=0, eval_cache=True,
                 leaves_per_step=1, gumbel=None, playout_cap=None, forced_playouts=None, surprise=False, search_value=False,
                 eval_symmetry=None, fpu=None, ownership=False, root_store=None, solver=False, resign=None, early_stop=None):
        if early_stop is not None and early_stop is not False and root_store is None:
            root_store = False
        self.root_store = check_root_store(root_store, eval_cache)
        self.ownership = check_ownership(ownership)
        self.resign = check_resign(resign, self.ownership)
        self.eval_symmetry = check_eval_symmetry(eval_symmetry, seed, game, evaluator)
        if not isinstance(surprise, (bool, np.bool_)):
            raise ValueError(f"surprise must be a bool (got {surprise!r})")
        self.surprise = bool(surprise)
        self.search_value = check_search_value(search_value)
        check_sims(sims, reuse_subtree)
        check_eval_cache(eval_cache)
        self.K = check_leaves_per_step(leaves_per_step)
        self.gumbel = check_gumbel(gumbel, reuse_subtree, self.K, dirichlet_eps)
        self.playout_cap = check_playout_cap(playout_cap, sims, reuse_subtree, self.K, gumbel)
        self.forced_playouts = check_forced_playouts(forced_playouts, reuse_subtree, self.K, gumbel)
        self.fpu = check_fpu(fpu, reuse_subtree, self.K, gumbel)
        self._reuse = bool(reuse_subtree)
        self.solver = check_solver(solver, reuse_subtree, self.K, gumbel, forced_playouts, fpu)
        self.early_stop = check_early_stop(early_stop, reuse_subtree, self.K, gumbel, playout_cap, forced_playouts, solver,
                                           self.root_store, surprise, search_value, ownership, resign)
        if evaluator.startswith("mlp_") and _GAMES[game] != GAME_TTT:
            raise ValueError(f"evaluator {evaluator!r}: the MLP evaluators serve tic-tac-toe only")
        _lib.require_gpu()
        L = _lib.lib()
        self.game = _GAMES[game]
        self.device = torch.device(device)
        self._streams = {}
        t_max = 9 if self.game == GAME_TTT else 64
        self.cfg = EngineCfg(self.game, n_games, sims, _EVALS[evaluator], c_puct, temp_moves, openings, rounds, t_max,
                             stagger, seed, game_id_base, n_games if game_id_stride is None else game_id_stride,
                             (_lib.ENGINE_REUSE_SUBTREE if reuse_subtree else 0) | (_lib.ENGINE_EVAL_CACHE if eval_cache else 0) |
                             (_lib.ENGINE_EVAL_CACHE_CARRY if eval_cache in (True, "carry") else 0) |
                             ((self.K - 1) << _lib.ENGINE_LEAVES_SHIFT),
                             dirichlet_alpha, dirichlet_eps, ttt_lanes)
        nbytes = L.bz_engine_workspace_bytes(C.byref(self.cfg))
        if nbytes < 0:
            raise RuntimeError(_lib.last_error())
        self.ws = torch.zeros(nbytes + 256, dtype=torch.uint8, device=self.device)
        self._pad = (-self.ws.data_ptr()) & 255
        h = C.c_void_p()
        _lib.check(L.bz_engine_create(C.byref(self.cfg), self.ws.data_ptr() + self._pad, nbytes, C.byref(h)))
        self.h = h
        self.lay = EngineLayout()
        _lib.check(L.bz_engine_get_layout(self.h, C.byref(self.lay)))
        self.B, self.sims, self.rounds, self.na, self.t_max = n_games, sims, rounds, self.lay.na, t_max
        self.size = _SIZES[self.game]
        self.net = net
        if net is not None:
            from .mlp import DeviceMLP
            if isinstance(net, DeviceMLP):
                if net.max_batch < n_games * self.K:
                    raise ValueError(f"DeviceMLP max_batch {net.max_batch} < n_games {n_games}" +
                                     (f" x leaves_per_step {self.K}" if self.K > 1 else ""))
                _lib.check(L.bz_engine_set_mlp(self.h, net.h))
            else:
                _lib.check(L.bz_engine_set_net(self.h, net.h))
        if self.gumbel is not None:
            gc = self.gumbel
            gbytes = L.bz_engine_gumbel_bytes(C.byref(self.cfg), gc.max_considered)
            if gbytes < 0:
                raise RuntimeError(_lib.last_error())
            self.gws = torch.zeros(gbytes + 256, dtype=torch.uint8, device=self.device)
            gpad = (-self.gws.data_ptr()) & 255
            self._call(L.bz_engine_set_gumbel, gc.max_considered, gc.scale, gc.maxvisit_init, gc.value_scale,
                       self.gws.data_ptr() + gpad, gbytes)
            if gc.interior == "gumbel":
                self._set_gumbel_interior(True)
        if self.playout_cap is not None:
            pc = self.playout_cap
            cbytes = L.bz_engine_playout_cap_bytes(C.byref(self.cfg))
            if cbytes < 0:
                raise RuntimeError(_lib.last_error())
            self.cws = torch.zeros(cbytes + 256, dtype=torch.uint8, device=self.device)
            self._cpad = (-self.cws.data_ptr()) & 255
            self._call(L.bz_engine_set_playout_cap, pc.fast_sims, pc.full_q, self.cws.data_ptr() + self._cpad, cbytes)
        if self.forced_playouts is not None:
            self._call(L.bz_engine_set_forced_playouts, self.forced_playouts.k, int(self.forced_playouts.prune))
        if self.fpu is not None:
            self._set_fpu(self.fpu)
        if self.solver:
            self._set_solver(True)
        if self.surprise:
            sbytes = L.bz_engine_surprise_bytes(C.byref(self.cfg))
            if sbytes < 0:
                raise RuntimeError(_lib.last_error())
            self.sws = torch.zeros(sbytes + 256, dtype=torch.uint8, device=self.device)
            self._spad = (-self.sws.data_ptr()) & 255
            self._sbytes = sbytes
            self._call(L.bz_engine_set_surprise, self.sws.data_ptr() + self._spad, sbytes)
        if self.eval_symmetry is not None:
            _lib.check(L.bz_engine_set_eval_symmetry(self.h, 1, self.eval_symmetry.seed))
        if self.search_value:
            vbytes = L.bz_engine_search_value_bytes(C.byref(self.cfg))
            if vbytes < 0:
                raise RuntimeError(_lib.last_error())
            self.vws = torch.zeros(vbytes + 256, dtype=torch.uint8, device=self.device)
            self._vpad = (-self.vws.data_ptr()) & 255
            self._call(L.bz_engine_set_search_value, self.vws.data_ptr() + self._vpad, vbytes)
        if self.root_store is not None:
            S, D = self.root_store
            rbytes = L.bz_engine_root_store_bytes(C.byref(self.cfg), S, D)
            if rbytes < 0:
                raise RuntimeError(_lib.last_error())
            if rbytes == 0:
                self.root_store = None
            else:
                self.rws = torch.empty(rbytes + 256, dtype=torch.uint8, device=self.device)
                rpad = (-self.rws.data_ptr()) & 255
                self._call(L.bz_engine_set_root_store, self.rws.data_ptr() + rpad, rbytes, S, D)
        if self.ownership:
            obytes = L.bz_engine_ownership_bytes(C.byref(self.cfg))
            if obytes < 0:
                raise RuntimeError(_lib.last_error())
            self.ows = torch.zeros(obytes + 256, dtype=torch.uint8, device=self.device)
            self._opad = (-self.ows.data_ptr()) & 255
            self._call(L.bz_engine_set_ownership, self.ows.data_ptr() + self._opad, obytes)
        if self.resign is not None:
            self._set_resign(self.resign)
        if self.early_stop is not None:
            self._set_early_stop(self.early_stop)

    def _view(self, off, dtype, shape):
        n = int(np.prod(shape)) * torch.empty((), dtype=dtype).element_size()
        o = self._pad + off
        return self.ws[o:o + n].view(dtype).view(*shape)

    def _stream(self):
        st = torch.cuda.current_stream(self.device)
        self._streams[st.cuda_stream] = st
        return st.cuda_stream

    def _call(self, fn, *args):
        with torch.cuda.device(self.device):
            _lib.check(fn(self.h, *args, self._stream()))

    def reset_games(self):
        self._call(_lib.lib().bz_engine_reset_games)

    def set_roots(self, own, opp, to_move):
# ... 151 lines not shown

    def search(self):
        if self.early_stop is not None and self.early_stop.host_exit and self.cfg.eval_kind != EVAL_EXTERNAL:
            with torch.cuda.device(self.device):
                _lib.check(_lib.lib().bz_engines_search((C.c_void_p * 1)(self.h), (C.c_void_p * 1)(self._stream()), 1, 16))
            return
        self._call(_lib.lib().bz_engine_search)

    def search_external(self, eval_fn):
        lb = self.leaf_buffers()

        def fill():
            lg, v = eval_fn(lb["own"], lb["opp"], lb["kind"])
            lb["logits"].copy_(lg.to(torch.float32).reshape(lb["logits"].shape))
            lb["value"].copy_(v.to(torch.float32).reshape(lb["value"].shape))
        self.root_begin(); fill(); self.expand_backup()
        self.root_noise()
        for s in range(0, self.sims, self.K):
            self.select(s); fill(); self.expand_backup()

    def root_begin(self):
        self._call(_lib.lib().bz_engine_root_begin)

    def root_noise(self):
        self._call(_lib.lib().bz_engine_root_noise)

    def select(self, sim_index):
        self._call(_lib.lib().bz_engine_select, sim_index)

    def evaluate(self):
        self._call(_lib.lib().bz_engine_evaluate)

    def expand_backup(self):
        self._call(_lib.lib().bz_engine_expand_backup)

    def play(self, restart=False):
        self._call(_lib.lib().bz_engine_play, int(restart))

    def reset_counters(self):
        self._call(_lib.lib().bz_engine_reset_counters)

    def status(self):
        a, f, e = C.c_int32(), C.c_int64(), C.c_int32()
        with torch.cuda.device(self.device):
            _lib.check(_lib.lib().bz_engine_status(self.h, self._stream(), C.byref(a), C.byref(f), C.byref(e)))
        if e.value:
            names = [n for bit, n in ((1, "edge arena overflow"), (2, "terminal root"), (4, "example buffer overflow"),
                                      (8, "walk deeper than the path buffer"),
                                      (16, "the evaluator returned a non-finite logit or value")) if e.value & bit]
            raise RuntimeError(f"bz_engine error flags 0x{e.value:x}: " + ", ".join(names))
        return a.value, f.value

    def root_stats(self):
        self._call(_lib.lib().bz_engine_root_stats)
        shp = (self.B, self.na)
        N = self._view(self.lay.root_N, torch.int32, shp).cpu().numpy().view(np.uint32)
        W = self._view(self.lay.root_W, torch.float32, shp).cpu().numpy()
        P = self._view(self.lay.root_P, torch.float32, shp).cpu().numpy()
        return N, W, P

    def root_policy_dev(self):
        pi = torch.empty((self.B, self.na), dtype=torch.float32, device=self.device)
        act = torch.empty(self.B, dtype=torch.int32, device=self.device)
        self._call(_lib.lib().bz_engine_root_policy, pi.data_ptr(), act.data_ptr())
        return pi, act

    def root_policy(self):
        pi, act = self.root_policy_dev()
        return pi.cpu().numpy(), act.cpu().numpy()

    def budgets(self):
        if self.playout_cap is None:
            raise RuntimeError("budgets(): the engine was built without playout_cap")
        self.drain()
        torch.cuda.current_stream(self.device).synchronize()
        return self.cws[self._cpad:self._cpad + 4 * self.B].view(torch.int32).cpu().numpy().view(np.uint32)

    def counters(self):
        self._call(_lib.lib().bz_engine_sum_counters)
        c = self._view(self.lay.counters, torch.int64, (24,)).cpu().numpy()
        names = _lib.COUNTER_NAMES if self.K > 1 else _lib.COUNTER_NAMES[:_lib.COUNTER_NAMES.index("n_collisions")]
        return dict(zip(names, (int(v) for v in c[:len(names)])))

    def root_store_counters(self):
        self._call(_lib.lib().bz_engine_sum_counters)
        c = self._view(self.lay.counters, torch.int64, (24,)).cpu().numpy()
        return {"n_seeded_evals": int(c[11]), "n_seeded_searches": int(c[12]), "n_root_saves": int(c[13])}

    def leaf_buffers(self):
        R = self.B * self.K
        return {"own": self._view(self.lay.leaf_own, torch.int64, (R,)),
                "opp": self._view(self.lay.leaf_opp, torch.int64, (R,)),
                "kind": self._view(self.lay.leaf_kind, torch.uint8, (R,)),
                "logits": self._view(self.lay.logits, torch.float32, (R, self.na)),
                "value": self._view(self.lay.value, torch.float32, (R,))}

    def positions(self):
        return (_u64(self._view(self.lay.g_own, torch.int64, (self.B,))),
                _u64(self._view(self.lay.g_opp, torch.int64, (self.B,))),
                self._view(self.lay.g_to_move, torch.int8, (self.B,)).cpu().numpy(),
                self._view(self.lay.g_state, torch.uint8, (self.B,)).cpu().numpy())

    def example_tensors(self):
        R, B, T = self.rounds, self.B, self.t_max
        return {"own": self._view(self.lay.ex_own, torch.int64, (R, B, T)),
                "opp": self._view(self.lay.ex_opp, torch.int64, (R, B, T)),
                "pi": self._view(self.lay.ex_pi, torch.float32, (R, B, T, self.na)),
                "z": self._view(self.lay.ex_z, torch.int8, (R, B, T)),
                "mover": self._view(self.lay.ex_mover, torch.int8, (R, B, T)),
                "act": self._view(self.lay.ex_act, torch.uint8, (R, B, T)),
                "len": self._view(self.lay.ex_len, torch.int32, (R, B)),
                "winner": self._view(self.lay.ex_winner, torch.int8, (R, B))}

    def example_block(self):
        o = self._pad + self.lay.ex_begin
        return self.ws[o:o + self.lay.ex_bytes]

    def surprise_rows(self):
        if not self.surprise:
            raise RuntimeError("surprise_rows(): the engine was built without surprise=True")
        n = self.rounds * self.B * self.t_max * 4
        o = self._spad + self._sbytes - ((n + 255) & ~255)
        return self.sws[o:o + n].view(torch.float32).view(self.rounds, self.B, self.t_max)

    def pack_surprise(self, out=None, cap_rows=None, append=False):
        cap = int(cap_rows or self.rounds * self.B * self.t_max)
        if out is None:
            assert not append
            out = torch.zeros(cap, dtype=torch.float32, device=self.device)
        self._call(_lib.lib().bz_engine_pack_surprise, out.data_ptr(), cap, int(append))
        return out

    def _packed_kl(self, n_rows):
        cap = self.rounds * self.B * self.t_max
        self.pack_examples(cap_rows=cap)
        return self.pack_surprise(cap_rows=cap)[:n_rows]

    def search_value_rows(self):
        if not self.search_value:
            raise RuntimeError("search_value_rows(): the engine was built without search_value=True")
        n = self.rounds * self.B * self.t_max * 4
        return self.vws[self._vpad:self._vpad + n].view(torch.float32).view(self.rounds, self.B, self.t_max)

    def pack_search_value(self, out=None, cap_rows=None, append=False):
        cap = int(cap_rows or self.rounds * self.B * self.t_max)
        if out is None:
            assert not append
            out = torch.zeros(cap, dtype=torch.float32, device=self.device)
        self._call(_lib.lib().bz_engine_pack_search_value, out.data_ptr(), cap, int(append))
        return out

    def _packed_q(self, n_rows):
        cap = self.rounds * self.B * self.t_max
        self.pack_examples(cap_rows=cap)
        return self.pack_search_value(cap_rows=cap)[:n_rows]

    def ownership_rows(self):
        if not self.ownership:
            raise RuntimeError("ownership_rows(): the engine was built without ownership=True")
        n = self.rounds * self.B * 8
        step = (n + 255) & ~255
        return tuple(self.ows[self._opad + k * step:self._opad + k * step + n].view(torch.int64).view(self.rounds, self.B)
                     for k in (0, 1))

    def pack_ownership(self, out=None, cap_rows=None, append=False):
        cap = int(cap_rows or self.rounds * self.B * self.t_max)
# ... 269 lines not shown
        check_ownership(ownership)
        check_resign(resign, ownership)
        check_solver(solver, engine_kwargs.get("reuse_subtree", False), leaves_per_step, gumbel, forced_playouts, fpu)
        eval_symmetry = check_eval_symmetry(eval_symmetry, engine_kwargs.get("seed", 0), game, evaluator)
        check_search_value(search_value)
        check_leaves_per_step(leaves_per_step)
        check_gumbel(gumbel, engine_kwargs.get("reuse_subtree", False), leaves_per_step, engine_kwargs.get("dirichlet_eps", 0.0))
        check_playout_cap(playout_cap, sims, engine_kwargs.get("reuse_subtree", False), leaves_per_step, gumbel)
        check_forced_playouts(forced_playouts, engine_kwargs.get("reuse_subtree", False), leaves_per_step, gumbel)
        check_fpu(fpu, engine_kwargs.get("reuse_subtree", False), leaves_per_step, gumbel)
        check_eval_cache(engine_kwargs.get("eval_cache", True))
        check_root_store(engine_kwargs.get("root_store"), engine_kwargs.get("eval_cache", True))
        self.run_ahead = run_ahead
        self.device = torch.device(device)
        self.sizes = [n_games // pipelines + (1 if i < n_games % pipelines else 0) for i in range(pipelines)]
        self.streams = list(streams) if streams is not None else pipeline_streams(self.device, pipelines)
        assert len(self.streams) == pipelines
        stride = n_games if game_id_stride is None else game_id_stride
        self.engines = [SelfPlayEngine(game, self.sizes[i], sims, evaluator, net, game_id_base=game_id_base + sum(self.sizes[:i]),
                                       game_id_stride=stride, device=device, leaves_per_step=leaves_per_step, gumbel=gumbel,
                                       playout_cap=playout_cap, forced_playouts=forced_playouts, surprise=surprise,
                                       search_value=search_value, eval_symmetry=eval_symmetry, fpu=fpu, ownership=ownership, solver=solver,
                                       resign=resign, **engine_kwargs)
                        for i in range(pipelines)]
        self.surprise, self.search_value, self.ownership = bool(surprise), bool(search_value), bool(ownership)
        e0 = self.engines[0]
        self.B, self.sims, self.na, self.t_max, self.rounds, self.size, self.game = n_games, sims, e0.na, e0.t_max, e0.rounds, e0.size, e0.game

    def _fork(self):
        cur = torch.cuda.current_stream(self.device)
        for st in self.streams:
            st.wait_stream(cur)

    def join(self):
        cur = torch.cuda.current_stream(self.device)
        for st in self.streams:
            cur.wait_stream(st)

    def sync(self):
        for st in self.streams:
            st.synchronize()

    def _each(self, fn):
        out = []
        for e, st in zip(self.engines, self.streams):
            with torch.cuda.stream(st):
                out.append(fn(e))
        return out

    def reset_games(self):
        self._fork()
        self._each(lambda e: e.reset_games())

    def step(self, restart=False):
        self._fork()
        n = len(self.engines)
        for e, st in zip(self.engines, self.streams):
            e._streams[st.cuda_stream] = st
        with torch.cuda.device(self.device):
            _lib.check(_lib.lib().bz_engines_step((C.c_void_p * n)(*[e.h for e in self.engines]),
                                                  (C.c_void_p * n)(*[st.cuda_stream for st in self.streams]), n,
                                                  int(restart), int(self.run_ahead)))

    def status(self):
        r = self._each(lambda e: e.status())
        return sum(a for a, _ in r), sum(f for _, f in r)

    def run_iteration(self, max_plies=None):
        self.reset_games()
        plies, limit = 0, max_plies or (12 if self.game == GAME_TTT else 140)
        while True:
            self.step(False)
            plies += 1
            if self.status()[0] == 0 or plies >= limit:
                return plies

    def reset_counters(self):
        self._each(lambda e: e.reset_counters())

    def budgets(self):
        self.sync()
        return np.concatenate([e.budgets() for e in self.engines])

    def root_store_counters(self):
        tot = {}
        for c in self._each(lambda e: e.root_store_counters()):
            for k, v in c.items():
                tot[k] = tot.get(k, 0) + v
        return tot

    def counters(self):
        tot = {}
        for c in self._each(lambda e: e.counters()):
            for k, v in c.items():
                tot[k] = tot.get(k, 0) + v
        return tot

    def example_blocks(self):
        self.join()
        return [e.example_block() for e in self.engines]

    def packed_capacity(self, games=None):
        return int((games if games is not None else self.rounds * self.B) * self.t_max)

    def pack_examples(self, out=None, cap_rows=None):
        cap = int(cap_rows or self.packed_capacity())
        if out is None:
            out = alloc_packed_block(self.na, cap, self.device)
        self.join()
        for i, e in enumerate(self.engines):
            e.pack_examples(out, cap, append=i > 0)
        return out

    def _pack_with_extras(self, out=None, cap_rows=None):
        cap = int(cap_rows or self.packed_capacity())
        if out is None:
            out = alloc_packed_block(self.na, cap, self.device)
        kl = torch.zeros(cap, dtype=torch.float32, device=self.device) if self.surprise else None
        q = torch.zeros(cap, dtype=torch.float32, device=self.device) if self.search_value else None
        own = tuple(torch.zeros(cap, dtype=torch.int64, device=self.device) for _ in range(2)) if self.ownership else None
        self.join()
        for i, e in enumerate(self.engines):
            e.pack_examples(out, cap, append=i > 0)
            if kl is not None:
                e.pack_surprise(kl, cap, append=i > 0)
            if q is not None:
                e.pack_search_value(q, cap, append=i > 0)
            if own is not None:
                e.pack_ownership(own, cap, append=i > 0)
        return out, kl, q, own

    def pack_examples_with_ownership(self, out=None, cap_rows=None):
        if not self.ownership:
            raise RuntimeError("pack_examples_with_ownership(): built without ownership=True")
        blk, _, _, own = self._pack_with_extras(out, cap_rows)
        return blk, own[0], own[1]

    def pack_examples_with_surprise(self, out=None, cap_rows=None):
        if not self.surprise:
            raise RuntimeError("pack_examples_with_surprise(): built without surprise=True")
        return self._pack_with_extras(out, cap_rows)[:2]

    def pack_examples_with_search_value(self, out=None, cap_rows=None):
        if not self.search_value:
            raise RuntimeError("pack_examples_with_search_value(): built without search_value=True")
        blk, _, q, _ = self._pack_with_extras(out, cap_rows)
        return blk, q

    def device_examples(self):
        blk, kl, q, own = self._pack_with_extras()
        ex = unpack_packed_block_device(blk)
        ex.kl = None if kl is None else kl[:len(ex)]
        ex.q = None if q is None else q[:len(ex)]
        if own is not None:
            ex.fown, ex.fopp = own[0][:len(ex)], own[1][:len(ex)]
        return ex

    def examples(self):
        blk, kl, q, own = self._pack_with_extras()
        ex = unpack_packed_block(blk)
        ex.kl = None if kl is None else kl[:len(ex)].cpu().numpy()
        ex.q = None if q is None else q[:len(ex)].cpu().numpy()
        if own is not None:
            ex.fown, ex.fopp = _u64(own[0][:len(ex)]), _u64(own[1][:len(ex)])
        return ex

# ... 63 lines not shown
```

include/bz_abi.h:

```cpp
#ifndef BZ_ABI_H
#define BZ_ABI_H
#include <stdint.h>

#ifdef __cplusplus
extern "C" {
#endif

#define BZ_ABI_VERSION 7

enum { BZ_OK = 0, BZ_EINVAL = 1, BZ_EILLEGAL_MOVE = 2, BZ_EHIP = 3, BZ_ENOMEM = 4, BZ_ENOGPU = 5,
       BZ_ESTATE = 6 };
enum { BZ_GAME_TTT = 0, BZ_GAME_REVERSI = 1, BZ_GAME_REVERSI6 = 2, BZ_GAME_REVERSI4 = 3 };
enum { BZ_EVAL_UNIFORM = 0, BZ_EVAL_HASH = 1, BZ_EVAL_NET_F32 = 2, BZ_EVAL_NET_BF16 = 3,
       BZ_EVAL_EXTERNAL = 4, BZ_EVAL_NET_FP8 = 5,
       BZ_EVAL_MLP_F32 = 6, BZ_EVAL_MLP_BF16 = 7 };
#define BZ_PASS_ACTION 64

int32_t bz_abi_version(void);
const char* bz_last_error(void);
const char* bz_build_info(void);
int32_t bz_device_count(void);

int32_t bz_reversi_legal(uint64_t own, uint64_t opp, int32_t size, uint64_t* legal);
int32_t bz_reversi_apply(uint64_t own, uint64_t opp, int32_t size, int32_t row, int32_t col,
// ... 99 lines not shown
    uint64_t game_id_stride;
    uint32_t flags;
    float dirichlet_alpha;
    float dirichlet_eps;
    int32_t ttt_lanes;
} bz_engine_cfg;
#define BZ_ENGINE_MAX_SIMS 8189
#define BZ_ENGINE_MAX_SIMS_REUSE 2045
#define BZ_ENGINE_REUSE_SUBTREE 1u
#define BZ_ENGINE_EVAL_CACHE 2u
#define BZ_ENGINE_EVAL_CACHE_CARRY 4u
#define BZ_ENGINE_LEAVES_SHIFT 8
#define BZ_ENGINE_LEAVES_MASK (31u << BZ_ENGINE_LEAVES_SHIFT)

typedef struct bz_engine_layout {
    int64_t ex_own, ex_opp;
    int64_t ex_pi;
    int64_t ex_z;
    int64_t ex_mover, ex_act;
    int64_t ex_len;
    int64_t ex_winner;
    int64_t root_N, root_W, root_P;
    int64_t leaf_own, leaf_opp;
    int64_t leaf_kind;
    int64_t logits, value;
    int64_t g_own, g_opp;
    int64_t g_to_move, g_state;
    int64_t counters;
    int32_t na, t_max;
    int64_t ex_begin, ex_bytes, ex_meta;
} bz_engine_layout;

int64_t bz_engine_workspace_bytes(const bz_engine_cfg* cfg);
int32_t bz_engine_create(const bz_engine_cfg* cfg, void* workspace, int64_t workspace_bytes,
                         bz_engine** out);
int32_t bz_engine_destroy(bz_engine* e);
int32_t bz_engine_get_layout(const bz_engine* e, bz_engine_layout* out);
int32_t bz_engine_set_net(bz_engine* e, bz_net* net);
int32_t bz_engine_set_mlp(bz_engine* e, bz_mlp* mlp);
int32_t bz_engine_debug_set_search_seq(bz_engine* e, uint32_t seq);
int32_t bz_engine_set_eval_symmetry(bz_engine* e, int32_t on, uint64_t seed);
int32_t bz_engine_reset_games(bz_engine* e, void* stream);
int32_t bz_engine_set_roots(bz_engine* e, const uint64_t* own, const uint64_t* opp,
                            const int8_t* to_move, void* stream);
int32_t bz_engine_search(bz_engine* e, void* stream);
int32_t bz_engine_root_begin(bz_engine* e, void* stream);
int32_t bz_engine_select(bz_engine* e, uint32_t sim_index, void* stream);
int32_t bz_engine_evaluate(bz_engine* e, void* stream);
int32_t bz_engine_expand_backup(bz_engine* e, void* stream);
int32_t bz_engine_root_noise(bz_engine* e, void* stream);
int32_t bz_engine_root_stats(bz_engine* e, void* stream);
int32_t bz_engine_play(bz_engine* e, int32_t restart, void* stream);
#define BZ_GUMBEL_MAX_CONSIDERED 64
int64_t bz_engine_gumbel_bytes(const bz_engine_cfg* cfg, int32_t max_considered);
int32_t bz_engine_set_gumbel(bz_engine* e, int32_t max_considered, float gumbel_scale, float maxvisit_init,
                             float value_scale, void* buf, int64_t buf_bytes, void* stream);
int32_t bz_gumbel_considered_visits(int32_t n_considered, int32_t sims, uint16_t* out);
int64_t bz_engine_gumbel_interior_bytes(const bz_engine_cfg* cfg);
int32_t bz_engine_set_gumbel_interior(bz_engine* e, int32_t on, void* buf, int64_t buf_bytes, void* stream);
int32_t bz_gumbel_interior_pick(const uint32_t* N, const float* W, const float* P, int32_t n, float v_node, float maxvisit_init,
                                float value_scale, float* p_out, float* score_out);
int64_t bz_engine_playout_cap_bytes(const bz_engine_cfg* cfg);
int32_t bz_engine_set_playout_cap(bz_engine* e, int32_t fast_sims, uint32_t full_q, void* buf, int64_t bytes, void* stream);
int32_t bz_playout_cap_budget(uint64_t seed, uint64_t gid, uint32_t moves_made, int32_t sims, int32_t fast_sims, uint32_t full_q);
int32_t bz_engine_set_forced_playouts(bz_engine* e, float k, int32_t prune, void* stream);
int32_t bz_engine_forced_playouts_check(const bz_engine_cfg* cfg, float k);
int32_t bz_forced_prune(const uint32_t* N, const float* W, const float* P, int32_t n, float c_puct, float k, uint32_t* N_out);
int64_t bz_engine_fpu_bytes(const bz_engine_cfg* cfg);
int32_t bz_engine_fpu_check(const bz_engine_cfg* cfg, float reduction, float root_reduction);
int32_t bz_engine_set_fpu(bz_engine* e, int32_t on, float reduction, float root_reduction, void* buf, int64_t bytes, void* stream);
uint32_t bz_fpu_mass(const uint32_t* N, const float* P, int32_t n);
float bz_fpu_value(const uint32_t* N, const float* P, int32_t n, float q_node, float reduction);
int64_t bz_engine_solver_bytes(const bz_engine_cfg* cfg);
int32_t bz_engine_solver_check(const bz_engine_cfg* cfg);
int32_t bz_engine_set_solver(bz_engine* e, int32_t on, void* buf, int64_t bytes, void* stream);
int32_t bz_engine_root_proven(bz_engine* e, int8_t* edge_out, int8_t* root_out, uint32_t* counts_out, void* stream);
int32_t bz_solver_node(const int8_t* vals, int32_t n);
int32_t bz_solver_pick(const uint32_t* N, const int8_t* vals, int32_t n, int32_t tau1, uint64_t draw);
int64_t bz_engine_early_stop_bytes(const bz_engine_cfg* cfg);
int32_t bz_engine_early_stop_check(const bz_engine_cfg* cfg);
int32_t bz_engine_set_early_stop(bz_engine* e, int32_t on, int32_t host_exit, void* buf, int64_t bytes, void* stream);
int32_t bz_engine_stopped(bz_engine* e, uint32_t* out, void* stream);
int32_t bz_early_stop_decided(const uint32_t* N, int32_t n, uint32_t left);
int64_t bz_engine_surprise_bytes(const bz_engine_cfg* cfg);
int32_t bz_engine_set_surprise(bz_engine* e, void* buf, int64_t bytes, void* stream);
int32_t bz_engine_pack_surprise(bz_engine* e, float* out, int64_t cap_rows, int32_t append_rows, void* stream);
int32_t bz_surprise_kl(const float* pi, const float* P, int32_t n, float* kl);
int64_t bz_surprise_resample_workspace_bytes(int64_t n);
int32_t bz_surprise_resample(const float* kl, const int64_t* game, const int32_t* ply, const uint64_t* own, const uint64_t* opp,
                             int64_t n, float uniform_frac, uint64_t seed, void* ws, int64_t ws_bytes, int32_t* count,
                             int64_t* idx_out, int64_t idx_cap, int64_t* n_out, void* stream);
int32_t bz_surprise_count(float kl, float mean, float uniform_frac, uint64_t seed, int64_t game, int32_t ply, uint64_t own,
                          uint64_t opp, int32_t* count);
int64_t bz_engine_search_value_bytes(const bz_engine_cfg* cfg);
int32_t bz_engine_set_search_value(bz_engine* e, void* buf, int64_t bytes, void* stream);
int32_t bz_engine_pack_search_value(bz_engine* e, float* out, int64_t cap_rows, int32_t append_rows, void* stream);
int32_t bz_root_value(const uint32_t* N, const float* W, int32_t n, float* q);
int32_t bz_value_targets(const float* q, const int8_t* z, const int8_t* mover, const int64_t* game, const int32_t* ply, int64_t n,
                         float lam, float q_mix, float* vt, uint64_t* status_dev, void* stream);
int32_t bz_value_targets_segment(const float* q, const int8_t* z, const int8_t* mover, int32_t T, float lam, float q_mix, float* vt);
typedef struct bz_merge_rows {
    uint64_t* own; uint64_t* opp; float* pi; int8_t* z; int8_t* mover; uint8_t* act; int64_t* game; int32_t* ply;
    float* vt;
    float* q; float* kl;
} bz_merge_rows;
int32_t bz_merge_group(const float* pi, const float* vt, const int8_t* z, const float* q, const float* kl, int32_t n, int32_t na,
                       float* pi_out, float* vt_out, int8_t* z_out, float* q_out, float* kl_out, int32_t* bad);
int64_t bz_merge_workspace_bytes(int64_t n, int32_t na);
int32_t bz_merge_positions(const bz_merge_rows* in, int64_t n, int32_t na, const int64_t* order, const int32_t* start,
                           const int32_t* dst, const int64_t* head, const int32_t* count, const int64_t* n_groups, void* ws,
                           int64_t ws_bytes, const bz_merge_rows* out, uint64_t* status_dev, void* stream);
int64_t bz_engine_ownership_bytes(const bz_engine_cfg* cfg);
int32_t bz_engine_set_ownership(bz_engine* e, void* buf, int64_t bytes, void* stream);
int32_t bz_engine_pack_ownership(bz_engine* e, uint64_t* fown_out, uint64_t* fopp_out, int64_t cap_rows, int32_t append_rows,
                                 void* stream);
int32_t bz_ownership_row(uint64_t fin_x, uint64_t fin_o, int32_t mover, uint64_t* t_own, uint64_t* t_opp);
#define BZ_RESIGN_KEY 0x72657369676E6564ULL
int64_t bz_engine_resign_bytes(const bz_engine_cfg* cfg);
int32_t bz_engine_set_resign(bz_engine* e, float threshold, int32_t consecutive, uint32_t playout_q, void* buf, int64_t bytes,
                             void* stream);
int32_t bz_engine_resign_rows(bz_engine* e, int8_t* side, int32_t* move, float* q, uint8_t* played_out, void* stream);
int32_t bz_resign_step(float q, float threshold, int32_t consecutive, int32_t streak_in, int32_t* streak_out);
int32_t bz_resign_playout(uint64_t seed, uint64_t gid, uint32_t playout_q);
int64_t bz_engine_root_store_bytes(const bz_engine_cfg* cfg, int32_t entries, int32_t plies);
int32_t bz_engine_set_root_store(bz_engine* e, void* buf, int64_t bytes, int32_t entries, int32_t plies, void* stream);
int32_t bz_engine_root_policy(bz_engine* e, float* pi, int32_t* action, void* stream);
#define BZ_ENGINE_ERR_EDGE_OVERFLOW 1
#define BZ_ENGINE_ERR_TERMINAL_ROOT 2
#define BZ_ENGINE_ERR_EXAMPLE_OVERFLOW 4
#define BZ_ENGINE_ERR_DEPTH 8
#define BZ_ENGINE_ERR_EVAL_NONFINITE 16
int32_t bz_engine_status(bz_engine* e, void* stream, int32_t* n_active, int64_t* games_finished,
                         int32_t* error_flags);
#define BZ_PACKED_MAGIC 0x425A50414B000001ULL
int64_t bz_examples_packed_bytes(int32_t na, int64_t cap_rows);
int32_t bz_engine_pack_examples(bz_engine* e, void* packed, int64_t packed_bytes, int64_t cap_rows, int32_t append,
                                void* stream);

int32_t bz_mcts_select(bz_engine* e, uint32_t sim_index, void* stream);
int32_t bz_mcts_expand_backup(bz_engine* e, void* stream);
int32_t bz_selfplay_run(bz_engine* e, int32_t restart, void* stream);
int32_t bz_engines_step(bz_engine* const* engines, void* const* streams, int32_t n, int32_t restart,
                        int32_t run_ahead_sims);
int32_t bz_engine_reset_counters(bz_engine* e, void* stream);
int32_t bz_engine_sum_counters(bz_engine* e, void* stream);

typedef struct bz_match bz_match;
#define BZ_MATCH_MAX_GAMES (1 << 24)
#define BZ_MATCH_ERR_ILLEGAL 0xC0000000u
#define BZ_MATCH_ERR_NO_ACTION 0xA0000000u
#define BZ_MATCH_ERR_SLOT_MASK 0x00FFFFFFu
typedef struct bz_match_layout {
    int64_t own, opp;
    int64_t to_move;
    int64_t active;
    int64_t winner;
    int64_t plies;
    int64_t a_colour;
    int64_t to_move_a, to_move_b;
    int64_t log_action, log_mover;
    int32_t n_games, max_plies;
} bz_match_layout;
typedef struct bz_match_hdr {
    int32_t ply;
    int32_t n_active;
    int32_t n_to_move_a, n_to_move_b;
// ... 120 lines not shown
```

Measured before the change: 243.1.

## Seed each search from the previous move's subtree and pace the remaining simulations

Adds a replay-seed kernel that finds the root's matching grandchild in the previous tree and compacts its subtree into the new tree. It rebuilds transposition-table entries and carries over visit counts as already-done simulations. A paced tree-step mode then spreads only the remaining simulations across the fixed step schedule, skipping walks for already-covered sims. This aims to cut network evaluations and tree walks per move. In exchange it adds an extra per-game kernel with LDS use and a fallback path. It only engages for plain search without Dirichlet noise, with the eval cache and compaction on, and for large batches unless forced on.

```diff
diff --git a/betazero_amd/_lib.py b/betazero_amd/_lib.py
--- a/betazero_amd/_lib.py
+++ b/betazero_amd/_lib.py
@@ -193,6 +193,8 @@
     "bz_engine_set_early_stop": (i32, [vp, i32, i32, vp, i64, vp]),
     "bz_engine_stopped": (i32, [vp, vp, vp]),
     "bz_early_stop_decided": (i32, [vp, i32, u32]),
+    "bz_engine_set_replay_seed": (i32, [vp, i32]),
+    "bz_pace_walk": (i32, [i32, i32, vp, vp]),
     "bz_engine_surprise_bytes": (i64, [C.POINTER(EngineCfg)]),
     "bz_engine_set_surprise": (i32, [vp, vp, i64, vp]),
     "bz_engine_pack_surprise": (i32, [vp, vp, i64, i32, vp]),
diff --git a/betazero_amd/csrc/bz_mcts.hip b/betazero_amd/csrc/bz_mcts.hip
--- a/betazero_amd/csrc/bz_mcts.hip
+++ b/betazero_amd/csrc/bz_mcts.hip
@@ -8,6 +8,7 @@
 #include "bz_fpu.h"
 #include "bz_solver.h"
 #include "bz_early_stop.h"
+#include "bz_pace.h"
 #include "bz_gumbel_interior.h"
 #include "bz_surprise.h"
 #include "bz_value.h"
@@ -51,7 +52,7 @@
     u64 leaf_legal; u32 leaf_node, leaf_info;
     u32 depth, n_nodes, n_edges, leaf_slot;
     u32 root_n, root_base;
-    u32 tt_gen, copy_src, copy_e0, last_gen, prev_nodes, pad[1];
+    u32 tt_gen, copy_src, copy_e0, last_gen, prev_nodes, seeded;
 };
 constexpr u32 kSrcPrev = 1u << 31;
 static_assert(sizeof(GameHot) == 64, "layout");
@@ -164,12 +165,13 @@
     kModeGfull = 1u << 5,
     kModeSolve = 1u << 6,
     kModeStop = 1u << 7,
+    kModePace = 1u << 8,
 };
 template <unsigned M>
 struct Mode {
     static constexpr bool leaf = (M & kModeLeaf) != 0, gumbel = (M & kModeGumbel) != 0, cap = (M & kModeCap) != 0,
                           forced = (M & kModeForced) != 0, fpu = (M & kModeFpu) != 0, gfull = (M & kModeGfull) != 0,
-                          solve = (M & kModeSolve) != 0, stop = (M & kModeStop) != 0;
+                          solve = (M & kModeSolve) != 0, stop = (M & kModeStop) != 0, pace = (M & kModePace) != 0;
     static_assert(!gfull || gumbel, "search mode: the Gumbel interior rule needs Gumbel root search");
     static_assert(!gumbel || !(cap || forced || fpu || solve),
                   "search mode: Gumbel root search combines with none of playout cap, forced playouts, FPU reduction and the solver");
@@ -177,6 +179,7 @@
     static_assert(!leaf || M == kModeLeaf, "search mode: leaf-parallel search combines with nothing");
     static_assert(!stop || !(leaf || gumbel || cap || forced || gfull || solve),
                   "search mode: early stop combines with FPU reduction and with nothing else");
+    static_assert(!pace || M == kModePace, "search mode: the paced step serves the plain search only");
 };
 struct ModeArgs {
     const GumbelDev* gm = nullptr;
@@ -1099,7 +1102,7 @@
 template <class G, unsigned M>
 __device__ __forceinline__ void tree_step_body(const EngineDev& E, const ModeArgs& A, int do_expand, int do_select, u32 sim_idx) {
     constexpr bool kGumbel = Mode<M>::gumbel, kCap = Mode<M>::cap, kForced = Mode<M>::forced, kFpu = Mode<M>::fpu, kGfull = Mode<M>::gfull,
-                   kSolve = Mode<M>::solve, kStop = Mode<M>::stop;
+                   kSolve = Mode<M>::solve, kStop = Mode<M>::stop, kPace = Mode<M>::pace;
     static_assert(!Mode<M>::leaf, "search mode: the leaf-parallel step is k_leaf_step's own body");
     constexpr int kGW = G::GW;
     const int t = blockIdx.x * blockDim.x + threadIdx.x;
@@ -1133,11 +1136,25 @@
         pin(nlegal); pin(rown); pin(ropp); pin(root_base); pin(pe0.eidx); pin(pe0.w0); pin(pe0.W);
         const bool active = state == 0 && kind != LEAF_NONE;
         bool walk = kCap ? (active && sim_idx < bud) : active;
+        [[maybe_unused]] u32 my_sim = sim_idx;
+        [[maybe_unused]] bool seeded_root = false;
+        if constexpr (kPace) {
+            const u32 sd = hot.seeded, r = sd == kPaceIdle ? 0u : (u32)E.sims - sd;
+            walk = state == 0 && pace_walks(sim_idx, r, (u32)E.sims);
+            my_sim = sd + pace_done(sim_idx, r, (u32)E.sims);
+            seeded_root = sd != 0u && leaf == 0u;
+        }
         st.mark(0);
         if (do_expand && (kind == LEAF_EVAL || kind == LEAF_TERMINAL || kind == LEAF_COPY)) {
             float v;
             u32 e0 = ne; int n = 0;
-            if (kind == LEAF_EVAL) {
+            if (kPace && kind == LEAF_EVAL && seeded_root) {
+                v = E.value[row];
+                if (sub == 0) {
+                    if (!(v >= -3.0e38f && v <= 3.0e38f)) atomicOr(&E.flags[FLAG_ERR], ERR_EVAL_NONFINITE);
+                    c.v[CNT_NET_LEAVES]++;
+                }
+            } else if (kind == LEAF_EVAL) {
                 LogitSrc ls; ls.kind = BZ_EVAL_EXTERNAL; ls.h = 0; ls.row = E.logits + (size_t)row * G::NA;
                 v = E.value[row];
                 if (sub == 0 && !(v >= -3.0e38f && v <= 3.0e38f)) atomicOr(&E.flags[FLAG_ERR], ERR_EVAL_NONFINITE);
@@ -1222,7 +1239,7 @@
                 u32 leaf2; int k2, depth; float tv;
                 LeafPos lpos; lpos.own = 0; lpos.opp = 0; lpos.legal = 0; lpos.info = 0; lpos.src = 0; lpos.src_e0 = 0;
                 RootRef root; root.own = rown; root.opp = ropp; root.tm = rtm; root.n = root_n;
-                root.sumN = sim_idx + root_base; root.has_pre = pre_ok; root.pre = re0; root.tt_gen = hot.tt_gen; root.prev_nodes = hot.prev_nodes;
+                root.sumN = (kPace ? my_sim : sim_idx) + root_base; root.has_pre = pre_ok; root.pre = re0; root.tt_gen = hot.tt_gen; root.prev_nodes = hot.prev_nodes;
                 PathHbm<kGW> sink; sink.p = path; sink.mine.eidx = 0; sink.mine.w0 = 0; sink.mine.W = 0.0f; sink.mine.pad = 0;
                 const float fslot = (kForced && (!kCap || bud >= (u32)E.sims)) ? A.fo->k : 0.0f;
                 dev_select<G, M>(E, g, sub, root, nn, leaf2, k2, depth, tv, c, sink, lpos, st, A, fslot, kFpu ? rw : 0.0f);
@@ -1265,6 +1282,11 @@
 template <class G>
 __global__ void __launch_bounds__(256) k_tree_step(EngineDev E, int do_expand, int do_select, u32 sim_idx) {
     tree_step_body<G, 0u>(E, ModeArgs{}, do_expand, do_select, sim_idx);
+}
+
+template <class G>
+__global__ void __launch_bounds__(256) k_pace_step(EngineDev E, int do_expand, int do_select, u32 sim_idx) {
+    tree_step_body<G, kModePace>(E, ModeArgs{}, do_expand, do_select, sim_idx);
 }
 
 template <class G>
@@ -2227,6 +2249,7 @@
     Node* nodes; Edge* edges; float* node_v; u64* tt;
 };
 constexpr int kCntSeededEvals = 11, kCntSeededSearches = 12, kCntStoreSaves = 13;
+constexpr int kCntReplaySeeds = 14, kCntReplaySims = 15;
 
 __device__ __forceinline__ u32 store_home(const StoreDev& St, u64 own, u64 opp) { return (u32)(hash_pos(own, opp) >> 20) & (u32)(St.n_idx - 1); }
 __device__ __forceinline__ int store_find(const StoreDev& St, u64 own, u64 opp, u64 epoch, u32* at) {
@@ -2391,6 +2414,150 @@
         St.mark[g] = gen;
         atomicAdd(reinterpret_cast<unsigned long long*>(E.counters) + kCntSeededSearches, 1ULL);
     }
+}
+
+template <class G>
+__global__ void __launch_bounds__(G::GW) k_replay_seed(EngineDev E, u32 gen, int do_seed, const u32* store_mark) {
+    constexpr int kGW = G::GW;
+    constexpr u32 kNone = 0xFFFFu;
+    extern __shared__ u32 s_map[];
+    uint16_t* s_par = reinterpret_cast<uint16_t*>(s_map + E.ncap);
+    uint16_t* s_ord = s_par + E.ncap;
+    const int g = blockIdx.x, sub = threadIdx.x;
+    GameHot* hot = E.hot + g;
+    const bool searching = E.g_state[g] == 0 && E.leaf_kind[g] == LEAF_EVAL;
+    const u32 pn = hot->prev_nodes;
+    u32 cand = ~0u;
+    const Node* sn = E.nodes_alt + (size_t)g * E.ncap;
+    const Edge* se = E.edges_alt + (size_t)g * E.ecap;
+    if (do_seed && searching && pn > 1u && pn <= (u32)E.ncap && !(store_mark && store_mark[g] == tt_gen_before(gen))) {
+        const u64 rown = E.g_own[g], ropp = E.g_opp[g];
+        const Node oroot = sn[0];
+        const u32 n0 = ((oroot.info & kTerm) || oroot.edge0 + (oroot.info & 0xFFu) > (u32)E.ecap) ? 0u : (oroot.info & 0xFFu);
+        for (u32 i = sub; i < n0; i += kGW) {
+            const Edge e = se[oroot.edge0 + i];
+            u32 ch = e_child(e.w3), N = e_N(e.w0);
+            if (!ch || ch >= pn || e_decided(e.w0)) continue;
+            const Node* cn = sn + ch;
+            if (cn->legal == 0 && (cn->info & 0xFFu) == 1u && cn->edge0 < (u32)E.ecap) {
+                const Edge pe = se[cn->edge0];
+                ch = e_child(pe.w3); N = e_N(pe.w0);
+                if (!ch || ch >= pn || e_decided(pe.w0)) continue;
+                cn = sn + ch;
+            }
+            const u32 ci = cn->info;
+            if (cn->own == rown && cn->opp == ropp && !(ci & kTerm) && (ci & 0xFFu) != 0u && N >= 2u) cand = ch | (N << kChildBits);
+        }
+    }
+    cand = group_min_u32<kGW>(cand);
+    if (cand == ~0u) {
+        if (sub == 0) hot->seeded = searching ? 0u : kPaceIdle;
+        return;
+    }
+    const u32 r_old = cand & kChildMask, seeded = (cand >> kChildBits) - 1u;
+    for (u32 i = r_old + sub; i < pn; i += kGW) s_par[i] = (uint16_t)kNone;
+    __syncthreads();
+    for (u32 i = r_old + sub; i < pn; i += kGW) {
+        const Node nd = sn[i];
+        const u32 n = ((nd.info & kTerm) || nd.edge0 + (nd.info & 0xFFu) > (u32)E.ecap) ? 0u : (nd.info & 0xFFu);
+        s_map[i] = n;
+        for (u32 j = 0; j < n; ++j) {
+            const u32 ch = e_child(se[nd.edge0 + j].w3);
+            if (ch > i && ch < pn) s_par[ch] = (uint16_t)i;
+        }
+    }
+    __syncthreads();
+    u32 nT = 0, eT = 0;
+    for (u32 i = r_old; i < pn; ++i) {
+        const u32 p = s_par[i], n = s_map[i];
+        const bool in = i == r_old || (p != kNone && s_map[p] != ~0u);
+        if (in) {
+            s_map[i] = nT | (eT << kChildBits);
+            s_ord[nT] = (uint16_t)i;
+            ++nT; eT += n;
+        } else {
+            s_map[i] = ~0u;
+        }
+    }
+    __syncthreads();
+    if (eT > (u32)E.ecap) {
+        if (sub == 0) hot->seeded = 0u;
+        return;
+    }
+    Node* dn = E.nodes + (size_t)g * E.ncap;
+    Edge* de = E.edges + (size_t)g * E.ecap;
+    const float* sv = E.node_v_alt + (size_t)g * E.ncap;
+    float* dv = E.node_v + (size_t)g * E.ncap;
+    u32 c_vis = 0, c_scored = 0, c_exp = 0, c_written = 0, root_sum = 0;
+    for (u32 k = sub; k < nT; k += kGW) {
+        const u32 i = s_ord[k];
+        const Node nd = sn[i];
+        const u32 e0n = s_map[i] >> kChildBits;
+        const u32 n = ((nd.info & kTerm) || nd.edge0 + (nd.info & 0xFFu) > (u32)E.ecap) ? 0u : (nd.info & 0xFFu);
+        u32 sumN = 0;
+        for (u32 j = 0; j < n; ++j) {
+            Edge e = se[nd.edge0 + j];
+            const u32 ch = e_child(e.w3);
+            if (ch) {
+                const u32 mc = ch < pn ? s_map[ch] : 0u;
+                e.w3 = e_nch(e.w0) ? mc : (mc & kChildMask);
+            }
+            sumN += e_N(e.w0);
+            de[e0n + j] = e;
+        }
+        dv[k] = sv[i];
+        if (k != 0u) {
+            Node out;
+            out.own = nd.own; out.opp = nd.opp; out.legal = nd.legal; out.edge0 = n ? e0n : 0u; out.info = nd.info;
+            dn[k] = out;
+        } else {
+            root_sum = sumN;
+        }
+        c_vis += sumN; c_scored += n * sumN; c_exp += n ? 1u : 0u; c_written += n;
+    }
+    root_sum = group_sum_u32<kGW>(root_sum);
+    group_fence();
+    u32 hits = 0, hits_prev = 0;
+    bool exact = root_sum == seeded;
+    for (u32 k = 1; exact && k < nT; ++k) {
+        const Node nd = sn[s_ord[k]];
+        if (nd.info & kTerm) continue;
+        u32 src = 0, src_e0 = 0;
+        if (tt_lookup_insert<kGW>(E, g, sub, nd.own, nd.opp, gen, pn, k, src, src_e0)) { ++hits; hits_prev += (src & kSrcPrev) ? 1u : 0u; }
+        else exact = false;
+    }
+    if (!exact) {
+        u64* tt = E.tt + (size_t)g * (size_t)E.tt_buckets * 16;
+        for (u32 k = sub; k < (u32)E.tt_buckets * 16u; k += kGW)
+            if (((u32)(tt[k] >> 32) >> kChildBits) == gen) tt[k] = 0ULL;
+        if (sub == 0) hot->seeded = 0u;
+        return;
+    }
+    c_vis = group_sum_u32<kGW>(c_vis); c_scored = group_sum_u32<kGW>(c_scored);
+    c_exp = group_sum_u32<kGW>(c_exp); c_written = group_sum_u32<kGW>(c_written);
+    if (sub == 0) {
+        const u32 rn = sn[r_old].info & 0xFFu;
+        dn[0].edge0 = 0; dn[0].info = (dn[0].info & ~0xFFu) | rn;
+        hot->n_nodes = nT; hot->n_edges = eT; hot->root_n = rn; hot->seeded = seeded;
+        atomicAdd(reinterpret_cast<unsigned long long*>(E.counters) + kCntReplaySeeds, 1ULL);
+        atomicAdd(reinterpret_cast<unsigned long long*>(E.counters) + kCntReplaySims, (unsigned long long)seeded);
+    }
+    u32 add = 0;
+    switch (sub) {
+    case CNT_SIMS: add = seeded; break;
+    case CNT_PATH_NODES: add = seeded + c_vis; break;
+    case CNT_CHILD_SCORED: add = c_scored; break;
+    case CNT_EDGES_BACKED: add = c_vis; break;
+    case CNT_EXPANDED: add = c_exp; break;
+    case CNT_CHILD_WRITTEN: add = c_written; break;
+    case CNT_ENV_STEPS: add = nT - 1u; break;
+    case CNT_CACHE_HITS: add = hits; break;
+    case CNT_CACHE_HITS_PREV: add = hits_prev; break;
+    default: break;
+    }
+    if (add)
+        __hip_atomic_fetch_add(reinterpret_cast<unsigned long long*>(E.cnt_slots) + (size_t)(g % E.n_cnt_slots) * CNT_N + sub,
+                               (unsigned long long)add, __ATOMIC_RELAXED, __HIP_MEMORY_SCOPE_AGENT);
 }
 
 }
@@ -2428,6 +2595,7 @@
     int64_t store_index_bytes;
     int sym_on;
     uint64_t sym_seed;
+    int replay_seed, paced, seed_from_prev, seed_src;
 };
 
 namespace {
@@ -2551,6 +2719,7 @@
     if (!e) { set_error("out of host memory"); return BZ_ENOMEM; }
     e->cfg = *cfg; e->net = nullptr; e->mlp = nullptr; e->bytes = o.total; e->pack_parity = 1; e->n_ahead = 0; e->search_seq = 0; e->eval_epoch = 0;
     e->sym_on = 0; e->sym_seed = 0;
+    e->replay_seed = 2; e->paced = 0; e->seed_from_prev = 0; e->seed_src = 0;
     e->gumbel = GumbelDev{};
     e->gin = GumbelInDev{};
     e->cap = CapDev{};
@@ -2656,6 +2825,22 @@
     return BZ_OK;
 }
 
+BZ_EXPORT int32_t bz_engine_set_replay_seed(bz_engine* e, int32_t mode) {
+    BZ_REQUIRE(e && mode >= 0 && mode <= 2, "bz_engine_set_replay_seed: null engine, or mode not 0 (off), 1 (on) or 2 (by the engine's size)");
+    e->replay_seed = mode;
+    return BZ_OK;
+}
+
+BZ_EXPORT int32_t bz_pace_walk(int32_t sims, int32_t r, uint8_t* walk, uint32_t* done) {
+    BZ_REQUIRE(walk && done && sims >= 1 && sims <= BZ_ENGINE_MAX_SIMS && r >= 0 && r <= sims,
+               "bz_pace_walk: null pointer, sims outside 1 .. 8189 or r outside 0 .. sims");
+    for (int32_t L = 0; L < sims; ++L) {
+        walk[L] = pace_walks((u32)L, (u32)r, (u32)sims) ? 1 : 0;
+        done[L] = pace_done((u32)L, (u32)r, (u32)sims);
+    }
+    return BZ_OK;
+}
+
 BZ_EXPORT int32_t bz_engine_debug_set_search_seq(bz_engine* e, uint32_t seq) {
     BZ_REQUIRE(e, "null engine");
     BZ_REQUIRE(seq < kTtGenMax - 1u, "bz_engine_debug_set_search_seq: 0 <= seq <= 2^19 - 3");
@@ -2722,6 +2907,8 @@
     }
     e->pack_parity = 1;
     e->fpu_done = 0;
+    e->paced = 0;
+    e->seed_src = e->seed_from_prev; e->seed_from_prev = 0;
     if (e->solve.root)
         BZ_HIP(hipMemsetAsync(e->solve.root, 0, (size_t)e->solve_bytes, (hipStream_t)stream));
     if (e->stop.stop_at) {
@@ -2740,11 +2927,12 @@
 
 static int32_t tree_step(bz_engine* e, int do_expand, int do_select, uint32_t sim_idx, void* stream) {
     ProfScope ps(do_select ? BZ_PROF_SELECT : BZ_PROF_EXPAND_BACKUP, stream);
-    const unsigned m = engine_mode(e);
+    const unsigned m = engine_mode(e) | (e->paced ? kModePace : 0u);
     if ((m & kModeFpu) && !do_select) sim_idx = (uint32_t)e->fpu_done;
 #define BZ_STEP(KERNEL, ...) BZ_DISPATCH_G(e, KERNEL, stream, __VA_ARGS__, do_expand, do_select, sim_idx); break
     switch (m) {
     case 0u: BZ_STEP(k_tree_step, e->dev);
+    case kModePace: BZ_STEP(k_pace_step, e->dev);
     case kModeLeaf: BZ_STEP(k_leaf_step, e->dev);
     case kModeGumbel: BZ_STEP(k_gumbel_step, e->dev, e->gumbel);
     case kModeGumbel | kModeGfull: BZ_STEP(k_gfull_step, e->dev, e->gumbel, e->gin);
@@ -2824,6 +3012,26 @@
 static bool search_is_fused(const bz_engine* e) {
     const int ek = e->cfg.eval_kind;
     return (ek == BZ_EVAL_UNIFORM || ek == BZ_EVAL_HASH) && !e->dev.reuse && !root_prep(e) && engine_mode(e) == 0u;
+}
+
+constexpr int kPaceAutoSlots = 1024;
+static int32_t paced_search(bz_engine* e, void* stream) {
+    const int from_prev = e->seed_src;
+    const bool plain = engine_mode(e) == 0u && !(e->dev.dir_eps > 0.0f) && !e->dev.reuse && !e->sym_on && e->dev.ecache == 2 &&
+                       net_eval(e->cfg.eval_kind) && e->cfg.game != BZ_GAME_TTT && e->dev.compact;
+    if (!plain || e->replay_seed == 0 || (e->replay_seed == 2 && e->dev.B <= kPaceAutoSlots)) return BZ_OK;
+    const size_t lds = (size_t)e->dev.ncap * 8;
+    const u32* mark = e->store.S > 0 ? e->store.mark : nullptr;
+#define BZ_SEED(G) hipLaunchKernelGGL(k_replay_seed<G>, dim3(e->dev.B), dim3(G::GW), lds, (hipStream_t)stream, e->dev, e->search_seq, from_prev, mark)
+    switch (e->cfg.game) {
+    case BZ_GAME_REVERSI6: BZ_SEED(Reversi6); break;
+    case BZ_GAME_REVERSI4: BZ_SEED(Reversi4); break;
+    default: BZ_SEED(Reversi); break;
+    }
+#undef BZ_SEED
+    BZ_LAUNCH_CHECK("k_replay_seed");
+    e->paced = 1;
+    return BZ_OK;
 }
 
 static int32_t store_save(bz_engine* e, void* stream) {
@@ -2863,6 +3071,7 @@
     BZ_REQUIRE(ek != BZ_EVAL_EXTERNAL, "bz_engine_search: BZ_EVAL_EXTERNAL callers drive the step API");
     int32_t rc;
     if ((rc = bz_engine_root_begin(e, stream)) != BZ_OK) return rc;
+    if ((rc = paced_search(e, stream)) != BZ_OK) return rc;
     if ((rc = bz_engine_evaluate(e, stream)) != BZ_OK) return rc;
     if (noise) {
         if ((rc = tree_step(e, 1, 0, 0, stream)) != BZ_OK) return rc;
@@ -2873,6 +3082,7 @@
         if ((rc = bz_engine_evaluate(e, stream)) != BZ_OK) return rc;
     }
     if ((rc = tree_step(e, 1, 0, 0, stream)) != BZ_OK) return rc;
+    e->seed_from_prev = e->paced;
     return store_save(e, stream);
 }
 
@@ -3710,6 +3920,7 @@
         steps = ns > steps ? ns : steps;
         Kmax = e->dev.K > Kmax ? e->dev.K : Kmax;
         if ((rc = bz_engine_root_begin(e, streams[i])) != BZ_OK) return rc;
+        if ((rc = paced_search(e, streams[i])) != BZ_OK) return rc;
         if ((rc = bz_engine_evaluate(e, streams[i])) != BZ_OK) return rc;
         if (root_prep(e)) {
             if ((rc = tree_step(e, 1, 0, 0, streams[i])) != BZ_OK) return rc;
@@ -3756,6 +3967,7 @@
         bz_engine* e = engines[i];
         if (!e || search_is_fused(e)) continue;
         if ((rc = tree_step(e, 1, 0, 0, streams[i])) != BZ_OK) return rc;
+        e->seed_from_prev = e->paced;
         if ((rc = store_save(e, streams[i])) != BZ_OK) return rc;
         if (play && (rc = bz_engine_play(e, restart, streams[i])) != BZ_OK) return rc;
     }
diff --git a/betazero_amd/csrc/bz_pace.h b/betazero_amd/csrc/bz_pace.h
--- /dev/null
+++ b/betazero_amd/csrc/bz_pace.h
@@ -0,0 +1,11 @@
+#pragma once
+#include "bz_math.h"
+
+namespace bz {
+
+BZ_HD u32 pace_done(u32 L, u32 r, u32 sims) { return (L * r) / sims; }
+BZ_HD bool pace_walks(u32 L, u32 r, u32 sims) { return pace_done(L + 1u, r, sims) > pace_done(L, r, sims); }
+
+constexpr u32 kPaceIdle = ~0u;
+
+}
diff --git a/betazero_amd/engine.py b/betazero_amd/engine.py
--- a/betazero_amd/engine.py
+++ b/betazero_amd/engine.py
@@ -170,6 +170,14 @@
 
 
 MAX_CONSIDERED = 64
+
+
+def check_replay_seed(replay_seed):
+    if replay_seed is None:
+        return None
+    if not isinstance(replay_seed, (bool, np.bool_)):
+        raise ValueError(f"replay_seed must be None, True or False (got {replay_seed!r})")
+    return bool(replay_seed)
 
 
 @dataclass(frozen=True)
@@ -421,7 +429,9 @@
                  seed=0, rounds=1, game_id_base=0, game_id_stride=None, device="cuda:0", stagger=0,
                  dirichlet_alpha=0.0, dirichlet_eps=0.0, reuse_subtree=False, ttt_lanes=0, eval_cache=True,
                  leaves_per_step=1, gumbel=None, playout_cap=None, forced_playouts=None, surprise=False, search_value=False,
-                 eval_symmetry=None, fpu=None, ownership=False, root_store=None, solver=False, resign=None, early_stop=None):
+                 eval_symmetry=None, fpu=None, ownership=False, root_store=None, solver=False, resign=None, early_stop=None,
+                 replay_seed=None):
+        self.replay_seed = check_replay_seed(replay_seed)
         if early_stop is not None and early_stop is not False and root_store is None:
             root_store = False
         self.root_store = check_root_store(root_store, eval_cache)
@@ -479,6 +489,8 @@
                 _lib.check(L.bz_engine_set_mlp(self.h, net.h))
             else:
                 _lib.check(L.bz_engine_set_net(self.h, net.h))
+        if self.replay_seed is not None:
+            _lib.check(L.bz_engine_set_replay_seed(self.h, int(self.replay_seed)))
         if self.gumbel is not None:
             gc = self.gumbel
             gbytes = L.bz_engine_gumbel_bytes(C.byref(self.cfg), gc.max_considered)
@@ -796,6 +808,15 @@
         names = _lib.COUNTER_NAMES if self.K > 1 else _lib.COUNTER_NAMES[:_lib.COUNTER_NAMES.index("n_collisions")]
         return dict(zip(names, (int(v) for v in c[:len(names)])))
 
+    def set_replay_seed(self, on=None):
+        self.replay_seed = check_replay_seed(on)
+        _lib.check(_lib.lib().bz_engine_set_replay_seed(self.h, 2 if self.replay_seed is None else int(self.replay_seed)))
+
+    def replay_seed_counters(self):
+        self._call(_lib.lib().bz_engine_sum_counters)
+        c = self._view(self.lay.counters, torch.int64, (24,)).cpu().numpy()
+        return {"n_replay_seeds": int(c[14]), "n_replay_sims": int(c[15])}
+
     def root_store_counters(self):
         self._call(_lib.lib().bz_engine_sum_counters)
         c = self._view(self.lay.counters, torch.int64, (24,)).cpu().numpy()
@@ -1231,6 +1252,13 @@
         self.sync()
         return np.concatenate([e.budgets() for e in self.engines])
 
+    def replay_seed_counters(self):
+        tot = {}
+        for c in self._each(lambda e: e.replay_seed_counters()):
+            for k, v in c.items():
+                tot[k] = tot.get(k, 0) + v
+        return tot
+
     def root_store_counters(self):
         tot = {}
         for c in self._each(lambda e: e.root_store_counters()):
diff --git a/include/bz_abi.h b/include/bz_abi.h
--- a/include/bz_abi.h
+++ b/include/bz_abi.h
@@ -205,6 +205,9 @@
 int32_t bz_engine_set_early_stop(bz_engine* e, int32_t on, int32_t host_exit, void* buf, int64_t bytes, void* stream);
 int32_t bz_engine_stopped(bz_engine* e, uint32_t* out, void* stream);
 int32_t bz_early_stop_decided(const uint32_t* N, int32_t n, uint32_t left);
+
+int32_t bz_engine_set_replay_seed(bz_engine* e, int32_t mode);
+int32_t bz_pace_walk(int32_t sims, int32_t r, uint8_t* walk, uint32_t* done);
 int64_t bz_engine_surprise_bytes(const bz_engine_cfg* cfg);
 int32_t bz_engine_set_surprise(bz_engine* e, void* buf, int64_t bytes, void* stream);
 int32_t bz_engine_pack_surprise(bz_engine* e, float* out, int64_t cap_rows, int32_t append_rows, void* stream);
```

After: 246.9, median of 6. 1.6% higher.
